# LIU-YUXI/SA-GNN

Hardware: AMD Instinct MI355X
Metric: spmm_edges_per_sec (higher is better)
Workload: dtype f32

## Files before the change

### include/sagnn.h

```cpp
#ifndef SAGNN_H
#define SAGNN_H

#include <stddef.h>
#include <stdint.h>

#ifdef __cplusplus
extern "C" {
#endif

#define SAGNN_VERSION 10400

enum {
  SAGNN_OK = 0,
  SAGNN_ERR_NULL = -1,
  SAGNN_ERR_DIM = -2,
  SAGNN_ERR_ALIGN = -3,
  SAGNN_ERR_CSR = -4,
  SAGNN_ERR_ARG = -5,
  SAGNN_ERR_WORKSPACE = -6,
  SAGNN_ERR_NOMEM = -7
};

int sagnn_version(void);

enum { SAGNN_ENGINE_F16X2 = 0, SAGNN_ENGINE_F32 = 1, SAGNN_ENGINE_VALU = 2 };
int sagnn_set_engine(int engine);
int sagnn_get_engine(void);
int sagnn_range_redo_count(int64_t* count, int reset);

size_t sagnn_last_error(char* buf, size_t cap);

int sagnn_profile_enable(int capacity);
int sagnn_profile_read(float* ms, int32_t* kind, int64_t* units_a, int64_t* units_b, int cap,
                       int* n_out);

int sagnn_csr_check_host(const int32_t* h_rowptr, const int32_t* h_colidx,
                         int64_t n_rows, int64_t n_src, int64_t nnz);

typedef struct sagnn_spmm_plan sagnn_spmm_plan;

typedef struct sagnn_spmm_tuning {
  int32_t short_thresh;
  int32_t long_thresh;
  int32_t chunk_edges;
  int32_t reserved;
} sagnn_spmm_tuning;

typedef struct sagnn_spmm_plan_info {
  int64_t n_rows, n_src, nnz;
  int64_t n_long_rows;
  int64_t n_chunks;
  int32_t short_thresh, long_thresh, chunk_edges;
  int32_t max_degree;
  int32_t on_device;
  int32_t weighted;
} sagnn_spmm_plan_info;

int sagnn_spmm_plan_create(const int32_t* h_rowptr, const int32_t* d_rowptr,
                           const int32_t* d_colidx, int64_t n_rows, int64_t n_src,
                           int64_t nnz, const sagnn_spmm_tuning* tuning ,
                           sagnn_spmm_plan** plan_out);
int sagnn_spmm_plan_destroy(sagnn_spmm_plan* plan);
int sagnn_spmm_plan_get_info(const sagnn_spmm_plan* plan, sagnn_spmm_plan_info* info);
int sagnn_spmm_plan_copy_chunks(const sagnn_spmm_plan* plan, int32_t* rows, int32_t* e_begin,
                                int32_t* e_end, int64_t cap);
int sagnn_spmm_plan_set_weights(sagnn_spmm_plan* plan, const float* d_weights);
size_t sagnn_spmm_workspace_bytes(const sagnn_spmm_plan* plan, int d);

int sagnn_spmm_f32(const sagnn_spmm_plan* plan, const float* X, int64_t ldx, int d,
                   const float* residual, int64_t ldr, float leaky, float* out, int64_t ldo,
                   const float* acc_in, int64_t ld_acc_in, float* acc_out, int64_t ld_acc_out,
                   void* workspace, size_t workspace_bytes, void* stream);

typedef struct sagnn_spmm_epilogue {
  float leaky;
  const float* residual; int64_t ldr;
  float* out; int64_t ldo;
  const float* acc_in; int64_t ld_acc_in;
  float* acc_out; int64_t ld_acc_out;
  uint8_t* mask_out;
  const uint8_t* mask_in;
  float* out2; int64_t ldo2; float slope2;
  const float* acc_in2; int64_t ld_acc_in2;
} sagnn_spmm_epilogue;

int sagnn_spmm_ex_f32(const sagnn_spmm_plan* plan, const float* X, int64_t ldx, int d,
                      const sagnn_spmm_epilogue* epilogue, void* workspace, size_t workspace_bytes,
                      void* stream);
int sagnn_mask_scale_f32(const float* g, int64_t ldg, const uint8_t* mask, float slope, float* out, int64_t ldo,
                         int64_t n_rows, int d, void* stream);

typedef struct sagnn_spmm_batch sagnn_spmm_batch;
int sagnn_spmm_batch_create(const sagnn_spmm_plan* const* plans_user, const sagnn_spmm_plan* const* plans_item,
                            int n_intervals, sagnn_spmm_batch** batch_out);
int sagnn_spmm_batch_destroy(sagnn_spmm_batch* batch);
size_t sagnn_spmm_batch_workspace_bytes(const sagnn_spmm_batch* batch, int d);

typedef struct sagnn_edge_drop {
  uint64_t seed;
  uint32_t step;
  uint32_t keep_threshold;
  float scale;
} sagnn_edge_drop;

int sagnn_spmm_drop_f32(const sagnn_spmm_plan* plan, const float* X, int64_t ldx, int d,
                        const sagnn_spmm_epilogue* epilogue, const sagnn_edge_drop* drop, uint32_t tag,
                        int rows_are_users, void* workspace, size_t workspace_bytes, void* stream);

int sagnn_spmm_plan_set_buckets(sagnn_spmm_plan* plan, const uint16_t* d_buckets, int32_t n_buckets);

typedef struct sagnn_edge_time {
  const float* te;
  int64_t stride_interval;
  int64_t stride_layer;
  int64_t stride_dir;
  int32_t n_buckets;
  float* dte;
  const sagnn_spmm_plan* adj_user;
  const sagnn_spmm_plan* adj_item;
  const sagnn_spmm_batch* adj_batch;
  void* adj_workspace;
  size_t adj_workspace_bytes;
} sagnn_edge_time;

int sagnn_spmm_time_batch_create(const sagnn_spmm_plan* const* adj_user, const sagnn_spmm_plan* const* adj_item,
                                 int n_intervals, sagnn_spmm_batch** batch_out);

int sagnn_spmm_time_f32(const sagnn_spmm_plan* plan, const float* X, int64_t ldx, int d,
                        const sagnn_spmm_epilogue* epilogue, const sagnn_edge_drop* drop, const sagnn_edge_time* time,
                        void* workspace, size_t workspace_bytes, void* stream);

typedef struct sagnn_gnn_side {
  const float* in;   int64_t ld_in,  slab_in;
  float*       out;  int64_t ld_out, slab_out;
  float*       scratch;
  uint8_t*     mask;
} sagnn_gnn_side;

enum { SAGNN_EDGES_PLAIN = 0, SAGNN_EDGES_DROP = 1, SAGNN_EDGES_TIME = 2 };

typedef struct sagnn_gnn_args {
  sagnn_gnn_side user, item;
  int d, n_layers;
  float leaky;
  int edges;
  const sagnn_edge_drop* drop;
  const sagnn_edge_time* time;
  int interval;
  void* workspace; size_t workspace_bytes;
} sagnn_gnn_args;

int sagnn_gnn_interval_f32(const sagnn_spmm_plan* plan_user, const sagnn_spmm_plan* plan_item, const sagnn_gnn_args* args,
                           void* stream);
int sagnn_gnn_interval_bwd_f32(const sagnn_spmm_plan* plan_user, const sagnn_spmm_plan* plan_item,
                               const sagnn_gnn_args* args, void* stream);
int sagnn_gnn_stack_f32(const sagnn_spmm_batch* batch, const sagnn_gnn_args* args, void* stream);
int sagnn_gnn_stack_bwd_f32(const sagnn_spmm_batch* batch, const sagnn_gnn_args* args, void* stream);

int sagnn_lstm_fwd_f32(const float* x, int64_t ld_n, int64_t ld_t, int64_t n, int t, int d, const float* W,
                       const float* b, float forget_bias, const float* drop_scale, float* h,
                       int64_t ld_h, void* stream);
int sagnn_lstm_fwd_state_f32(const float* x, int64_t ld_n, int64_t ld_t, int64_t n, int t, int d,
                             const float* W, const float* b, float forget_bias, const float* drop_scale,
                             const float* h_init, int64_t ld_hi, const float* c_init, float* h, int64_t ld_h,
                             float* c_final, void* stream);
int sagnn_layernorm_td_f32(const float* x, int64_t ld_n, int64_t ld_t, int64_t n, int t, int d,
                           const float* gamma, const float* beta, float eps, float* y,
                           int64_t ld_y, void* stream);
int sagnn_mhsa_mean_f32(const float* x, int64_t ld_n, int64_t ld_t, int64_t n, int t, int d, int heads,
                        const float* Wq, const float* bq, const float* Wk, const float* bk,
                        const float* Wv, const float* bv, float* out, int64_t ld_out,
                        void* stream);
size_t sagnn_mhsa_wide_workspace_bytes(int64_t n, int t, int d);
int sagnn_mhsa_mean_wide_f32(const float* x, int64_t ld_n, int64_t ld_t, int64_t n, int t, int d, int heads,
                             const float* Wq, const float* bq, const float* Wk, const float* bk, const float* Wv,
                             const float* bv, float* out, int64_t ld_out, void* workspace, size_t workspace_bytes,
                             void* stream);
size_t sagnn_ln_mhsa_mean_workspace_bytes(int64_t n, int t, int d, int heads);
int sagnn_ln_mhsa_mean_f32(const float* x, int64_t ld_n, int64_t ld_t, int64_t n, int t, int d, int heads,
                           const float* ln_gamma, const float* ln_beta, float ln_eps, const float* Wq,
                           const float* bq, const float* Wk, const float* bk, const float* Wv, const float* bv,
                           float* out, int64_t ld_out, void* workspace, size_t workspace_bytes, void* stream);
int sagnn_interval_fusion_f32(const float* x, int64_t ld_n, int64_t ld_t, int64_t n, int t, int d, int heads,
                              const float* lstm_W, const float* lstm_b, float forget_bias,
                              const float* ln_gamma, const float* ln_beta, float ln_eps,
                              const float* Wq, const float* bq, const float* Wk, const float* bk,
                              const float* Wv, const float* bv, float* out, int64_t ld_out,
                              void* workspace, size_t workspace_bytes, void* stream);
size_t sagnn_interval_fusion_workspace_bytes(int64_t n, int t, int d);

int sagnn_lstm_fwd_train_f32(const float* x, int64_t ld_n, int64_t ld_t, int64_t n, int t, int d,
                             const float* W, const float* b, float forget_bias, const float* drop_scale,
                             float* h, int64_t ld_h, float* gates, float* cell, void* stream);
int sagnn_attn_bwd_f32(float* qkv, const float* g_out, int64_t ld_g, int64_t n, int t, int d, int heads,
                       void* stream);
int sagnn_layernorm_td_bwd_f32(const float* h, int64_t ld_h, const float* dy, int64_t ld_dy, int64_t n, int t,
                               int d, const float* gamma, float eps, float* dh, int64_t ld_dh, float* dgamma,
                               float* dbeta, void* stream);
int sagnn_lstm_bwd_step_f32(const float* gates, const float* cell, const float* dh_ext, int64_t ld_dhe,
                            const float* drop_scale, const float* dh_rec, int64_t ld_dhr, const float* dc_in,
                            float* dgates, float* dc_out, int64_t n, int t, int d, int ts, void* stream);
int sagnn_attn_bwd_front_supported(int d, int t, int heads);
int sagnn_attn_bwd_front_f32(const float* x, int64_t ld_n, int64_t ld_t, int64_t n, int t, int d, int heads,
                             const float* ln_gamma, const float* ln_beta, float ln_eps, int apply_ln,
                             const float* Wq, const float* bq, const float* Wk, const float* bk, const float* Wv,
                             const float* bv, const float* g_out, int64_t ld_g, float* dqkv, float* y_out,
                             void* stream);
int sagnn_attn_bwd_tail_supported(int d);
int sagnn_attn_bwd_tail_f32(float* y, const float* dqkv, int64_t rows, int d, const float* Wqkv, float* dWqkv,
                            float* dbqkv, void* stream);
int sagnn_lstm_bwd_supported(int d);
int sagnn_lstm_bwd_f32(const float* x, int64_t ld_n, int64_t ld_t, const float* h, const float* gates,
                       const float* cell, const float* dh_ext, int64_t ld_dhe, const float* drop_scale,
                       const float* W, float* dx, float* dW, float* db, int64_t n, int t, int d, void* stream);
size_t sagnn_lstm_bwd_workspace_bytes(int64_t n, int t, int d);
int sagnn_lstm_bwd_ws_f32(const float* x, int64_t ld_n, int64_t ld_t, const float* h, const float* gates,
                          const float* cell, const float* dh_ext, int64_t ld_dhe, const float* drop_scale,
                          const float* W, float* dx, float* dW, float* db, int64_t n, int t, int d, void* workspace,
                          size_t workspace_bytes, void* stream);

int sagnn_leaky_add_f32(const float* a, const float* b, float* out, float leaky, int64_t count, void* stream);
int sagnn_pair_score_f32(const float* U, int64_t ldu, const float* I, int64_t ldi, const float* S, int64_t lds,
                         const float* A, int64_t lda, const int32_t* uids, const int32_t* iids,
                         const int32_t* locs, float leaky, float* out, int64_t n_pairs, int d, void* stream);

int sagnn_pair_score_bwd_f32(const float* U, int64_t ldu, const float* I, int64_t ldi, const float* S, int64_t lds,
                             const float* A, int64_t lda, const int32_t* uids, const int32_t* iids,
                             const int32_t* locs, float leaky, const float* g, float* dU, float* dI, float* dS,
                             float* dA, int64_t n_pairs, int d, void* stream);
int sagnn_prod_leaky_sum_f32(const float* X, int64_t ldx, const float* Y, int64_t ldy, const int32_t* uids,
                             const int32_t* iids, float leaky, float* out, int64_t n_pairs, int d, void* stream);
int sagnn_prod_leaky_sum_bwd_f32(const float* X, int64_t ldx, const float* Y, int64_t ldy, const int32_t* uids,
                                 const int32_t* iids, float leaky, const float* g, float* dX, float* dY,
                                 int64_t n_pairs, int d, void* stream);
int sagnn_meta_features_f32(const float* F, int64_t ldf, const float* V, int64_t ldv, const int32_t* uids,
                            float* out, int64_t n, int d, void* stream);
int sagnn_meta_features_bwd_f32(const float* F, int64_t ldf, const float* V, int64_t ldv, const int32_t* uids,
                                const float* dm, float* dF, float* dV, int64_t n, int d, void* stream);
int sagnn_leaky_f32(const float* a, const float* g, float* out, float leaky, int64_t count, int backward,
                    void* stream);
int sagnn_rowdot_sigmoid_f32(const float* A, int64_t lda, const float* w3, const float* b3, float* out, int64_t n,
                             int k, void* stream);
int sagnn_rowdot_sigmoid_bwd_f32(const float* A, int64_t lda, const float* w3, const float* w, const float* dw,
                                 float* dA, int64_t ldda, float* dw3, float* db3, int64_t n, int k, void* stream);
int sagnn_hinge_f32(const float* pos, const float* neg, const float* wp, const float* wn, const float* sp,
                    const float* sn, float scale, float* loss, float* dpos, float* dneg, float* dwp, float* dwn,
                    int64_t n, void* stream);

int sagnn_mul_f32(const float* a, const float* b, float* out, int64_t count, void* stream);

int sagnn_adam_step_f32(float* param, const float* grad, float* m, float* v, int64_t count, float lr,
                        float beta1, float beta2, float eps, float l2, int64_t step, void* stream);

int sagnn_adam_multi_f32(int n_tensors, float* const* params, const float* const* grads, float* const* m,
                         float* const* v, const int64_t* counts, const float* l2, float lr, float beta1,
                         float beta2, float eps, int64_t step, void* stream);

int sagnn_dense_nn_f32(const float* X, int64_t ldx, int64_t n, int din, int dout, const float* W,
                       const float* bias, float* Y, int64_t ldy, int accumulate, void* stream);
int sagnn_dense_tn_f32(const float* X, int64_t ldx, const float* G, int64_t ldg, int64_t n, int din,
                       int dout, float* dW, float* db, void* stream);
int sagnn_dense_tn_seg_f32(const float* X, int64_t ldx, int64_t x_seg, const float* G, int64_t ldg, int64_t g_seg,
                           int64_t seg_rows, int n_seg, int din, int dout, float* dW, float* db, void* stream);

size_t sagnn_score_topk_workspace_bytes(int64_t n_queries, int64_t n_items, int d, int k);
int sagnn_score_topk_f32(const float* Q, int64_t ldq, const float* I, int64_t ldi, int64_t n_queries, int64_t n_items,
                         int d, int k, const int32_t* excl_rowptr, const int32_t* excl_items, const int32_t* target,
                         int32_t* topk_items, float* topk_scores, int64_t* target_rank, void* workspace,
                         size_t workspace_bytes, void* stream);

int sagnn_candidate_rank_f32(const float* U, int64_t ldu, const float* I, int64_t ldi, const float* S, int64_t lds,
                             const float* A, int64_t lda, const int32_t* uids, const int32_t* cand, int64_t ldc,
                             const int32_t* target, float leaky, int64_t n_rows, int C, int d, int64_t* rank,
                             float* scores, int64_t ld_scores, void* stream);

int sagnn_sample_train_i32(const int32_t* bat_ids, int64_t n_batch, int64_t n_slots, const int64_t* seq_ptr,
                           const int32_t* seq_items, const int64_t* ban_ptr, const int32_t* ban_items, int64_t n_users,
                           int64_t n_items, int train_sample_num, int pred_num, int pos_length, const int64_t* pair_off,
                           int64_t n_pairs, uint64_t seed, int64_t step, int32_t* uids, int32_t* iids,
                           int32_t* uLocs_seq, int64_t* seg_begin, int32_t* seg_len, void* stream);
int sagnn_sample_ssl_i32(const int32_t* bat_ids, int64_t n_batch, int n_intervals, const int64_t* sub_ptr,
                         const int32_t* sub_items, int64_t n_users, int ssl_num, const int64_t* ssl_off, int64_t n_out,
                         uint64_t seed, int64_t step, int32_t* uids, int32_t* iids, int32_t* uLocs_seq, void* stream);
int sagnn_seq_sum_f32(const float* fi, int64_t ldf, int64_t n_items, const float* pos_embed, int64_t ldp,
                      int pos_length, const int32_t* seq_items, int64_t n_flat, const int64_t* seg_begin,
                      const int32_t* seg_len, int64_t n_slots, int d, float* seq_tok, float* pos_tok, int64_t ldo,
                      void* stream);
int sagnn_seq_sum_bwd_f32(const float* g_seq, const float* g_pos, int64_t ldg, const int32_t* seq_items, int64_t n_flat,
                          const int64_t* seg_begin, const int32_t* seg_len, int64_t n_slots, int pos_length, int d,
                          float* d_fi, int64_t ld_dfi, int64_t n_items, float* d_pos, int64_t ld_dpos, void* stream);

int sagnn_rows_mark_i32(const int32_t* ids, int64_t n_ids, int64_t n_rows, uint8_t* flags, void* stream);
int sagnn_rows_mark_seg_i32(const int32_t* seq_items, int64_t n_flat, const int64_t* seg_begin, const int32_t* seg_len,
                            int64_t n_slots, int max_len, int64_t n_rows, uint8_t* flags, void* stream);
size_t sagnn_rows_compact_workspace_bytes(int64_t n_rows);
int sagnn_rows_compact_i32(uint8_t* flags, int64_t n_rows, int32_t* rows, int64_t cap, int32_t* count, void* workspace,
                           size_t workspace_bytes, void* stream);
int sagnn_rows_gather_f32(const float* x, int64_t ld_n, int64_t ld_t, int64_t n_rows, int t, int d, const int32_t* rows,
                          int64_t cap, const int32_t* count, float* out, void* stream);
int sagnn_rows_scatter_f32(const float* src, const int32_t* rows, int64_t cap, const int32_t* count, int t, int d,
                           float* dst, int64_t ld_n, int64_t ld_t, int64_t n_rows, void* stream);

int sagnn_seq_attn_supported(int d, int heads, int pos_length);
int sagnn_seq_gather_f32(const float* fi, int64_t ldf, int64_t n_items, const float* pos_embed, int64_t ldp,
                         int pos_length, const int32_t* seq_items, int64_t n_flat, const int32_t* seq_pos,
                         const int64_t* seg_begin, const int32_t* seg_len, int64_t n_slots, int d, float* seq_slab,
                         float* pos_slab, int64_t ldo, void* stream);
int sagnn_seq_gather_bwd_f32(const float* g_seq, const float* g_pos, int64_t ldg, const int32_t* seq_items,
                             int64_t n_flat, const int32_t* seq_pos, const int64_t* seg_begin, const int32_t* seg_len,
                             int64_t n_slots, int pos_length, int d, float* d_fi, int64_t ld_dfi, int64_t n_items,
                             float* d_pos, int64_t ld_dpos, void* stream);
int sagnn_seq_attn_f32(const float* qkv, const int32_t* seg_len, int64_t n_slots, int pos_length, int d, int heads,
                       float* ctx, void* stream);
int sagnn_seq_attn_bwd_f32(const float* qkv, const float* g_ctx, const int32_t* seg_len, int64_t n_slots,
                           int pos_length, int d, int heads, float* dqkv, void* stream);
int sagnn_seq_pool_f32(const float* x, int64_t ldx, const int32_t* seg_len, int64_t n_slots, int pos_length, int d,
                       float* out, int64_t ldo, void* stream);
int sagnn_seq_pool_bwd_f32(const float* g, int64_t ldg, const int32_t* seg_len, int64_t n_slots, int pos_length, int d,
                           float* dx, int64_t ldx, void* stream);

size_t sagnn_softmax_loss_workspace_bytes(int64_t n_queries, int64_t n_items, int d);
int sagnn_softmax_loss_f32(const float* Q, int64_t ldq, const float* I, int64_t ldi, int64_t n_queries, int64_t n_items,
                           int d, const int32_t* target, float inv_temp, float scale, const int64_t* excl_ptr,
                           const int32_t* excl_items, const int32_t* excl_row, int64_t n_lists, float* loss, float* lse,
                           float* tscore, void* workspace, size_t workspace_bytes, void* stream);
int sagnn_softmax_loss_bwd_f32(const float* Q, int64_t ldq, const float* I, int64_t ldi, int64_t n_queries,
                               int64_t n_items, int d, const int32_t* target, float inv_temp, float scale,
                               const int64_t* excl_ptr, const int32_t* excl_items, const int32_t* excl_row,
                               int64_t n_lists, const float* lse, const float* g, float* dQ, int64_t lddq, float* dI,
                               int64_t lddi, void* workspace, size_t workspace_bytes, void* stream);

#ifdef __cplusplus
}
#endif
#endif
```

### sa-gnn_amd/_lib.py

```python
from __future__ import annotations

import ctypes
import os
from ctypes import POINTER, c_char_p, c_float, c_int, c_int32, c_int64, c_size_t, c_uint32, c_uint64, c_void_p

_HERE = os.path.dirname(os.path.abspath(__file__))
LIB_PATH = os.environ.get("SAGNN_LIB") or os.path.join(_HERE, "lib", "libsagnn.so")


class SagnnError(RuntimeError):
    def __init__(self, code: int, msg: str):
        super().__init__(f"libsagnn error {code}: {msg}")
        self.code = code


class Tuning(ctypes.Structure):
    _fields_ = [("short_thresh", c_int32), ("long_thresh", c_int32), ("chunk_edges", c_int32),
                ("reserved", c_int32)]


class SpmmEpilogue(ctypes.Structure):
    _fields_ = [("leaky", c_float), ("residual", c_void_p), ("ldr", c_int64), ("out", c_void_p),
                ("ldo", c_int64), ("acc_in", c_void_p), ("ld_acc_in", c_int64), ("acc_out", c_void_p),
                ("ld_acc_out", c_int64), ("mask_out", c_void_p), ("mask_in", c_void_p),
                ("out2", c_void_p), ("ldo2", c_int64), ("slope2", c_float), ("acc_in2", c_void_p),
                ("ld_acc_in2", c_int64)]


class EdgeDropArgs(ctypes.Structure):
    _fields_ = [("seed", c_uint64), ("step", c_uint32), ("keep_threshold", c_uint32), ("scale", c_float)]


class EdgeTimeArgs(ctypes.Structure):
    _fields_ = [("te", c_void_p), ("stride_interval", c_int64), ("stride_layer", c_int64), ("stride_dir", c_int64),
                ("n_buckets", c_int32), ("dte", c_void_p), ("adj_user", c_void_p), ("adj_item", c_void_p),
                ("adj_batch", c_void_p), ("adj_workspace", c_void_p), ("adj_workspace_bytes", c_size_t)]


class GnnSide(ctypes.Structure):
    _fields_ = [("in_", c_void_p), ("ld_in", c_int64), ("slab_in", c_int64), ("out", c_void_p), ("ld_out", c_int64),
                ("slab_out", c_int64), ("scratch", c_void_p), ("mask", c_void_p)]


EDGES_PLAIN, EDGES_DROP, EDGES_TIME = 0, 1, 2


class GnnArgs(ctypes.Structure):
    _fields_ = [("user", GnnSide), ("item", GnnSide), ("d", c_int), ("n_layers", c_int), ("leaky", c_float),
                ("edges", c_int), ("drop", POINTER(EdgeDropArgs)), ("time", POINTER(EdgeTimeArgs)), ("interval", c_int),
                ("workspace", c_void_p), ("workspace_bytes", c_size_t)]


class PlanInfo(ctypes.Structure):
    _fields_ = [("n_rows", c_int64), ("n_src", c_int64), ("nnz", c_int64),
                ("n_long_rows", c_int64), ("n_chunks", c_int64), ("short_thresh", c_int32),
                ("long_thresh", c_int32), ("chunk_edges", c_int32), ("max_degree", c_int32),
                ("on_device", c_int32), ("weighted", c_int32)]


SIGNATURES = {
    "sagnn_version": (c_int, []),
    "sagnn_set_engine": (c_int, [c_int]),
    "sagnn_get_engine": (c_int, []),
    "sagnn_range_redo_count": (c_int, [POINTER(c_int64), c_int]),
    "sagnn_last_error": (c_size_t, [c_char_p, c_size_t]),
    "sagnn_profile_enable": (c_int, [c_int]),
    "sagnn_profile_read": (c_int, [c_void_p, c_void_p, c_void_p, c_void_p, c_int, POINTER(c_int)]),
    "sagnn_csr_check_host": (c_int, [c_void_p, c_void_p, c_int64, c_int64, c_int64]),
    "sagnn_spmm_plan_create": (c_int, [c_void_p, c_void_p, c_void_p, c_int64, c_int64, c_int64,
                                       POINTER(Tuning), POINTER(c_void_p)]),
    "sagnn_spmm_plan_destroy": (c_int, [c_void_p]),
    "sagnn_spmm_plan_get_info": (c_int, [c_void_p, POINTER(PlanInfo)]),
    "sagnn_spmm_plan_set_weights": (c_int, [c_void_p, c_void_p]),
    "sagnn_spmm_plan_copy_chunks": (c_int, [c_void_p, c_void_p, c_void_p, c_void_p, c_int64]),
    "sagnn_spmm_workspace_bytes": (c_size_t, [c_void_p, c_int]),
    "sagnn_spmm_f32": (c_int, [c_void_p, c_void_p, c_int64, c_int, c_void_p, c_int64, c_float,
                               c_void_p, c_int64, c_void_p, c_int64, c_void_p, c_int64, c_void_p,
                               c_size_t, c_void_p]),
    "sagnn_spmm_ex_f32": (c_int, [c_void_p, c_void_p, c_int64, c_int, POINTER(SpmmEpilogue), c_void_p, c_size_t,
                                  c_void_p]),
    "sagnn_mask_scale_f32": (c_int, [c_void_p, c_int64, c_void_p, c_float, c_void_p, c_int64, c_int64, c_int, c_void_p]),
    "sagnn_spmm_batch_create": (c_int, [c_void_p, c_void_p, c_int, POINTER(c_void_p)]),
    "sagnn_spmm_batch_destroy": (c_int, [c_void_p]),
    "sagnn_spmm_batch_workspace_bytes": (c_size_t, [c_void_p, c_int]),
    "sagnn_gnn_interval_f32": (c_int, [c_void_p, c_void_p, POINTER(GnnArgs), c_void_p]),
    "sagnn_gnn_interval_bwd_f32": (c_int, [c_void_p, c_void_p, POINTER(GnnArgs), c_void_p]),
    "sagnn_gnn_stack_f32": (c_int, [c_void_p, POINTER(GnnArgs), c_void_p]),
    "sagnn_gnn_stack_bwd_f32": (c_int, [c_void_p, POINTER(GnnArgs), c_void_p]),
    "sagnn_spmm_drop_f32": (c_int, [c_void_p, c_void_p, c_int64, c_int, POINTER(SpmmEpilogue), POINTER(EdgeDropArgs),
                                    c_uint32, c_int, c_void_p, c_size_t, c_void_p]),
    "sagnn_spmm_plan_set_buckets": (c_int, [c_void_p, c_void_p, c_int32]),
    "sagnn_spmm_time_batch_create": (c_int, [c_void_p, c_void_p, c_int, POINTER(c_void_p)]),
    "sagnn_spmm_time_f32": (c_int, [c_void_p, c_void_p, c_int64, c_int, POINTER(SpmmEpilogue), POINTER(EdgeDropArgs),
                                    POINTER(EdgeTimeArgs), c_void_p, c_size_t, c_void_p]),
    "sagnn_lstm_fwd_train_f32": (c_int, [c_void_p, c_int64, c_int64, c_int64, c_int, c_int, c_void_p, c_void_p, c_float,
                                         c_void_p, c_void_p, c_int64, c_void_p, c_void_p, c_void_p]),
    "sagnn_mhsa_wide_workspace_bytes": (c_size_t, [c_int64, c_int, c_int]),
    "sagnn_ln_mhsa_mean_workspace_bytes": (c_size_t, [c_int64, c_int, c_int, c_int]),
    "sagnn_ln_mhsa_mean_f32": (c_int, [c_void_p, c_int64, c_int64, c_int64, c_int, c_int, c_int, c_void_p, c_void_p,
                                       c_float, c_void_p, c_void_p, c_void_p, c_void_p, c_void_p, c_void_p, c_void_p,
                                       c_int64, c_void_p, c_size_t, c_void_p]),
    "sagnn_mhsa_mean_wide_f32": (c_int, [c_void_p, c_int64, c_int64, c_int64, c_int, c_int, c_int, c_void_p, c_void_p,
                                         c_void_p, c_void_p, c_void_p, c_void_p, c_void_p, c_int64, c_void_p, c_size_t,
                                         c_void_p]),
    "sagnn_attn_bwd_f32": (c_int, [c_void_p, c_void_p, c_int64, c_int64, c_int, c_int, c_int, c_void_p]),
    "sagnn_layernorm_td_bwd_f32": (c_int, [c_void_p, c_int64, c_void_p, c_int64, c_int64, c_int, c_int, c_void_p,
                                           c_float, c_void_p, c_int64, c_void_p, c_void_p, c_void_p]),
    "sagnn_lstm_bwd_step_f32": (c_int, [c_void_p, c_void_p, c_void_p, c_int64, c_void_p, c_void_p, c_int64, c_void_p,
                                        c_void_p, c_void_p, c_int64, c_int, c_int, c_int, c_void_p]),
    "sagnn_attn_bwd_front_supported": (c_int, [c_int, c_int, c_int]),
    "sagnn_attn_bwd_front_f32": (c_int, [c_void_p, c_int64, c_int64, c_int64, c_int, c_int, c_int, c_void_p, c_void_p,
                                         c_float, c_int, c_void_p, c_void_p, c_void_p, c_void_p, c_void_p, c_void_p,
                                         c_void_p, c_int64, c_void_p, c_void_p, c_void_p]),
    "sagnn_attn_bwd_tail_supported": (c_int, [c_int]),
    "sagnn_attn_bwd_tail_f32": (c_int, [c_void_p, c_void_p, c_int64, c_int, c_void_p, c_void_p, c_void_p, c_void_p]),
    "sagnn_lstm_bwd_supported": (c_int, [c_int]),
    "sagnn_lstm_bwd_f32": (c_int, [c_void_p, c_int64, c_int64, c_void_p, c_void_p, c_void_p, c_void_p, c_int64, c_void_p,
                                   c_void_p, c_void_p, c_void_p, c_void_p, c_int64, c_int, c_int, c_void_p]),
    "sagnn_lstm_bwd_workspace_bytes": (c_size_t, [c_int64, c_int, c_int]),
    "sagnn_lstm_bwd_ws_f32": (c_int, [c_void_p, c_int64, c_int64, c_void_p, c_void_p, c_void_p, c_void_p, c_int64, c_void_p,
                                      c_void_p, c_void_p, c_void_p, c_void_p, c_int64, c_int, c_int, c_void_p, c_size_t, c_void_p]),
    "sagnn_leaky_add_f32": (c_int, [c_void_p, c_void_p, c_void_p, c_float, c_int64, c_void_p]),
    "sagnn_pair_score_f32": (c_int, [c_void_p, c_int64, c_void_p, c_int64, c_void_p, c_int64, c_void_p, c_int64,
                                     c_void_p, c_void_p, c_void_p, c_float, c_void_p, c_int64, c_int, c_void_p]),
    "sagnn_pair_score_bwd_f32": (c_int, [c_void_p, c_int64, c_void_p, c_int64, c_void_p, c_int64, c_void_p, c_int64,
                                         c_void_p, c_void_p, c_void_p, c_float, c_void_p, c_void_p, c_void_p, c_void_p,
                                         c_void_p, c_int64, c_int, c_void_p]),
    "sagnn_prod_leaky_sum_f32": (c_int, [c_void_p, c_int64, c_void_p, c_int64, c_void_p, c_void_p, c_float, c_void_p,
                                         c_int64, c_int, c_void_p]),
    "sagnn_prod_leaky_sum_bwd_f32": (c_int, [c_void_p, c_int64, c_void_p, c_int64, c_void_p, c_void_p, c_float,
                                             c_void_p, c_void_p, c_void_p, c_int64, c_int, c_void_p]),
    "sagnn_meta_features_f32": (c_int, [c_void_p, c_int64, c_void_p, c_int64, c_void_p, c_void_p, c_int64, c_int,
                                        c_void_p]),
    "sagnn_meta_features_bwd_f32": (c_int, [c_void_p, c_int64, c_void_p, c_int64, c_void_p, c_void_p, c_void_p,
                                            c_void_p, c_int64, c_int, c_void_p]),
    "sagnn_leaky_f32": (c_int, [c_void_p, c_void_p, c_void_p, c_float, c_int64, c_int, c_void_p]),
    "sagnn_rowdot_sigmoid_f32": (c_int, [c_void_p, c_int64, c_void_p, c_void_p, c_void_p, c_int64, c_int, c_void_p]),
    "sagnn_rowdot_sigmoid_bwd_f32": (c_int, [c_void_p, c_int64, c_void_p, c_void_p, c_void_p, c_void_p, c_int64,
                                             c_void_p, c_void_p, c_int64, c_int, c_void_p]),
    "sagnn_hinge_f32": (c_int, [c_void_p, c_void_p, c_void_p, c_void_p, c_void_p, c_void_p, c_float, c_void_p,
                                c_void_p, c_void_p, c_void_p, c_void_p, c_int64, c_void_p]),
    "sagnn_mul_f32": (c_int, [c_void_p, c_void_p, c_void_p, c_int64, c_void_p]),
    "sagnn_adam_step_f32": (c_int, [c_void_p, c_void_p, c_void_p, c_void_p, c_int64, c_float, c_float, c_float,
                                    c_float, c_float, c_int64, c_void_p]),
    "sagnn_adam_multi_f32": (c_int, [c_int, c_void_p, c_void_p, c_void_p, c_void_p, c_void_p, c_void_p, c_float, c_float,
                                     c_float, c_float, c_int64, c_void_p]),
    "sagnn_dense_nn_f32": (c_int, [c_void_p, c_int64, c_int64, c_int, c_int, c_void_p, c_void_p, c_void_p, c_int64,
                                   c_int, c_void_p]),
    "sagnn_dense_tn_f32": (c_int, [c_void_p, c_int64, c_void_p, c_int64, c_int64, c_int, c_int, c_void_p, c_void_p,
                                   c_void_p]),
    "sagnn_dense_tn_seg_f32": (c_int, [c_void_p, c_int64, c_int64, c_void_p, c_int64, c_int64, c_int64, c_int, c_int, c_int,
                                       c_void_p, c_void_p, c_void_p]),
    "sagnn_lstm_fwd_f32": (c_int, [c_void_p, c_int64, c_int64, c_int64, c_int, c_int, c_void_p, c_void_p,
                                   c_float, c_void_p, c_void_p, c_int64, c_void_p]),
    "sagnn_lstm_fwd_state_f32": (c_int, [c_void_p, c_int64, c_int64, c_int64, c_int, c_int, c_void_p, c_void_p, c_float,
                                         c_void_p, c_void_p, c_int64, c_void_p, c_void_p, c_int64, c_void_p, c_void_p]),
    "sagnn_layernorm_td_f32": (c_int, [c_void_p, c_int64, c_int64, c_int64, c_int, c_int, c_void_p, c_void_p,
                                       c_float, c_void_p, c_int64, c_void_p]),
    "sagnn_mhsa_mean_f32": (c_int, [c_void_p, c_int64, c_int64, c_int64, c_int, c_int, c_int, c_void_p,
                                    c_void_p, c_void_p, c_void_p, c_void_p, c_void_p, c_void_p,
                                    c_int64, c_void_p]),
    "sagnn_interval_fusion_f32": (c_int, [c_void_p, c_int64, c_int64, c_int64, c_int, c_int, c_int, c_void_p,
                                          c_void_p, c_float, c_void_p, c_void_p, c_float, c_void_p,
                                          c_void_p, c_void_p, c_void_p, c_void_p, c_void_p, c_void_p,
                                          c_int64, c_void_p, c_size_t, c_void_p]),
    "sagnn_interval_fusion_workspace_bytes": (c_size_t, [c_int64, c_int, c_int]),
    "sagnn_score_topk_workspace_bytes": (c_size_t, [c_int64, c_int64, c_int, c_int]),
    "sagnn_score_topk_f32": (c_int, [c_void_p, c_int64, c_void_p, c_int64, c_int64, c_int64, c_int, c_int, c_void_p,
                                     c_void_p, c_void_p, c_void_p, c_void_p, c_void_p, c_void_p, c_size_t, c_void_p]),
    "sagnn_candidate_rank_f32": (c_int, [c_void_p, c_int64, c_void_p, c_int64, c_void_p, c_int64, c_void_p, c_int64,
                                         c_void_p, c_void_p, c_int64, c_void_p, c_float, c_int64, c_int, c_int, c_void_p,
                                         c_void_p, c_int64, c_void_p]),
    "sagnn_sample_train_i32": (c_int, [c_void_p, c_int64, c_int64, c_void_p, c_void_p, c_void_p, c_void_p, c_int64, c_int64,
                                       c_int, c_int, c_int, c_void_p, c_int64, c_uint64, c_int64, c_void_p, c_void_p,
                                       c_void_p, c_void_p, c_void_p, c_void_p]),
    "sagnn_sample_ssl_i32": (c_int, [c_void_p, c_int64, c_int, c_void_p, c_void_p, c_int64, c_int, c_void_p, c_int64,
                                     c_uint64, c_int64, c_void_p, c_void_p, c_void_p, c_void_p]),
    "sagnn_seq_sum_f32": (c_int, [c_void_p, c_int64, c_int64, c_void_p, c_int64, c_int, c_void_p, c_int64, c_void_p,
                                  c_void_p, c_int64, c_int, c_void_p, c_void_p, c_int64, c_void_p]),
    "sagnn_seq_sum_bwd_f32": (c_int, [c_void_p, c_void_p, c_int64, c_void_p, c_int64, c_void_p, c_void_p, c_int64, c_int,
                                      c_int, c_void_p, c_int64, c_int64, c_void_p, c_int64, c_void_p]),
    "sagnn_rows_mark_i32": (c_int, [c_void_p, c_int64, c_int64, c_void_p, c_void_p]),
    "sagnn_rows_mark_seg_i32": (c_int, [c_void_p, c_int64, c_void_p, c_void_p, c_int64, c_int, c_int64, c_void_p, c_void_p]),
    "sagnn_rows_compact_workspace_bytes": (c_size_t, [c_int64]),
    "sagnn_rows_compact_i32": (c_int, [c_void_p, c_int64, c_void_p, c_int64, c_void_p, c_void_p, c_size_t, c_void_p]),
    "sagnn_rows_gather_f32": (c_int, [c_void_p, c_int64, c_int64, c_int64, c_int, c_int, c_void_p, c_int64, c_void_p,
                                      c_void_p, c_void_p]),
    "sagnn_rows_scatter_f32": (c_int, [c_void_p, c_void_p, c_int64, c_void_p, c_int, c_int, c_void_p, c_int64, c_int64,
                                       c_int64, c_void_p]),
    "sagnn_seq_attn_supported": (c_int, [c_int, c_int, c_int]),
    "sagnn_seq_gather_f32": (c_int, [c_void_p, c_int64, c_int64, c_void_p, c_int64, c_int, c_void_p, c_int64, c_void_p,
                                     c_void_p, c_void_p, c_int64, c_int, c_void_p, c_void_p, c_int64, c_void_p]),
    "sagnn_seq_gather_bwd_f32": (c_int, [c_void_p, c_void_p, c_int64, c_void_p, c_int64, c_void_p, c_void_p, c_void_p,
                                         c_int64, c_int, c_int, c_void_p, c_int64, c_int64, c_void_p, c_int64, c_void_p]),
    "sagnn_seq_attn_f32": (c_int, [c_void_p, c_void_p, c_int64, c_int, c_int, c_int, c_void_p, c_void_p]),
    "sagnn_seq_attn_bwd_f32": (c_int, [c_void_p, c_void_p, c_void_p, c_int64, c_int, c_int, c_int, c_void_p, c_void_p]),
    "sagnn_seq_pool_f32": (c_int, [c_void_p, c_int64, c_void_p, c_int64, c_int, c_int, c_void_p, c_int64, c_void_p]),
    "sagnn_seq_pool_bwd_f32": (c_int, [c_void_p, c_int64, c_void_p, c_int64, c_int, c_int, c_void_p, c_int64, c_void_p]),
    "sagnn_softmax_loss_workspace_bytes": (c_size_t, [c_int64, c_int64, c_int]),
    "sagnn_softmax_loss_f32": (c_int, [c_void_p, c_int64, c_void_p, c_int64, c_int64, c_int64, c_int, c_void_p, c_float,
                                       c_float, c_void_p, c_void_p, c_void_p, c_int64, c_void_p, c_void_p, c_void_p,
                                       c_void_p, c_size_t, c_void_p]),
    "sagnn_softmax_loss_bwd_f32": (c_int, [c_void_p, c_int64, c_void_p, c_int64, c_int64, c_int64, c_int, c_void_p, c_float,
                                           c_float, c_void_p, c_void_p, c_void_p, c_int64, c_void_p, c_void_p, c_void_p,
                                           c_int64, c_void_p, c_int64, c_void_p, c_size_t, c_void_p]),
}


_lib = None


def load() -> ctypes.CDLL:
    global _lib
    if _lib is not None:
        return _lib
    if not os.path.exists(LIB_PATH):
        raise ImportError(
            f"{LIB_PATH} not found: build it with `python -c 'import __graft_entry__ as g; "
            "g.build()'` (or `make -C sa-gnn_amd/csrc`). There is no fallback path.")
    lib = ctypes.CDLL(LIB_PATH)
    lib.sagnn_version.restype = c_int
    if lib.sagnn_version() < 10400:
        raise ImportError(f"{LIB_PATH} is libsagnn {lib.sagnn_version()}: this binding needs >= 10400 (sagnn_gnn_args)")
    for name, (res, args) in SIGNATURES.items():
        fn = getattr(lib, name)
        fn.restype = res
        fn.argtypes = args
    _lib = lib
    return lib


def last_error() -> str:
    buf = ctypes.create_string_buffer(1024)
    load().sagnn_last_error(buf, 1024)
    return buf.value.decode("utf-8", "replace")


def check(rc: int) -> None:
    if rc != 0:
        raise SagnnError(rc, last_error())
```

### sa-gnn_amd/csrc/spmm.hip

```cpp
#include <float.h>

#include <algorithm>
#include <new>
#include <type_traits>
#include <vector>

#include "common.h"
#include "philox.h"

namespace {

constexpr int kWave = 64;
constexpr int kBlock = 256;
constexpr int kWavesPerBlock = kBlock / kWave;
constexpr int kRowsPerWave = 16;
constexpr int64_t kSmallRows = 262144;
constexpr int kUnroll = 8;

struct Epilogue {
  const float* residual;
  int64_t ldr;
  const float* acc_in;
  int64_t ld_acc_in;
  float* out;
  int64_t ldo;
  float* acc_out;
  int64_t ld_acc_out;
  float leaky;
  uint8_t* mask_out;
  const uint8_t* mask_in;
  float* out2;
  int64_t ldo2;
  float slope2;
  int mask_stride;
  const float* acc_in2;
  int64_t ld_acc_in2;
};

__device__ __forceinline__ float4 ld4(const float* p) {
  return *reinterpret_cast<const float4*>(p);
}
__device__ __forceinline__ void st4(float* p, float4 v) { *reinterpret_cast<float4*>(p) = v; }
typedef float f32x4_t __attribute__((ext_vector_type(4)));
__device__ __forceinline__ float4 ld4s(const float* p) {
#ifndef SAGNN_PLAIN_STREAMS
  const f32x4_t v = __builtin_nontemporal_load(reinterpret_cast<const f32x4_t*>(p));
  return make_float4(v.x, v.y, v.z, v.w);
#else
  return ld4(p);
#endif
}
__device__ __forceinline__ void st4s(float* p, float4 v) {
#ifndef SAGNN_PLAIN_STREAMS
  const f32x4_t w = {v.x, v.y, v.z, v.w};
  __builtin_nontemporal_store(w, reinterpret_cast<f32x4_t*>(p));
#else
  st4(p, v);
#endif
}
__device__ __forceinline__ int ldi_s(const int32_t* p) {
#ifndef SAGNN_PLAIN_STREAMS
  return __builtin_nontemporal_load(p);
#else
  return *p;
#endif
}
__device__ __forceinline__ float ldf_s(const float* p) {
#ifndef SAGNN_PLAIN_STREAMS
  return __builtin_nontemporal_load(p);
#else
  return *p;
#endif
}
__device__ __forceinline__ int ldb_s(const uint16_t* p) {
#ifndef SAGNN_PLAIN_STREAMS
  return __builtin_nontemporal_load(p);
#else
  return *p;
#endif
}
__device__ __forceinline__ void add4(float4& a, const float4& b) {
  a.x += b.x;
  a.y += b.y;
  a.z += b.z;
  a.w += b.w;
}

struct RowDrop {
  uint32_t k0, k1, step, thresh, tag;
  int rows_users;
  float scale;
};
struct BatchDrop {
  RowDrop r;
  uint32_t tag_i;
};

__device__ __forceinline__ RowDrop seg_drop(const BatchDrop& b, int dir, int k) {
  RowDrop r = b.r;
  r.tag = (dir ? b.tag_i : r.tag) | ((uint32_t)k << 8);
  r.rows_users = !dir;
  return r;
}

template <bool WEIGHTED>
__device__ __forceinline__ void acc4(float4& a, float w, const float4& v) {
  if constexpr (WEIGHTED) {
    a.x = fmaf(w, v.x, a.x);
    a.y = fmaf(w, v.y, a.y);
    a.z = fmaf(w, v.z, a.z);
    a.w = fmaf(w, v.w, a.w);
  } else {
    add4(a, v);
  }
}

template <bool DROP>
__device__ __forceinline__ int keep_edge(const RowDrop& dr, int row, int idx) {
  if constexpr (DROP) {
    const uint32_t u = dr.rows_users ? (uint32_t)row : (uint32_t)idx;
    const uint32_t i = dr.rows_users ? (uint32_t)idx : (uint32_t)row;
    const sagnn::Word4 w = sagnn::philox4x32_10(sagnn::Word4{u, i, dr.tag, dr.step}, dr.k0, dr.k1);
    return w.x < dr.thresh ? idx : -1;
  } else {
    return idx;
  }
}

template <bool DROP>
__device__ __forceinline__ float4 drop_scale(const RowDrop& dr, float4 s) {
  if constexpr (DROP) return make_float4(dr.scale * s.x, dr.scale * s.y, dr.scale * s.z, dr.scale * s.w);
  else return s;
}

struct RowTime {
  const uint16_t* bucket;
  const float* te;
};
struct BatchTime {
  const uint16_t* const* buckets;
  const float* te;
  int64_t s_k, s_dir;
};
__device__ __forceinline__ RowTime seg_time(const BatchTime& t, int seg, int dir, int k) {
  return RowTime{t.buckets[seg], t.te + (int64_t)k * t.s_k + (int64_t)dir * t.s_dir};
}
__device__ __forceinline__ RowTime seg_time(const RowTime& t, int, int, int) { return t; }

template <class T>
struct KernelArg { using type = T; };
template <class T>
struct KernelArg<T*> { using type = T* __restrict__; };
template <class Want, class... A>
constexpr bool kHas = (std::is_same_v<Want, A> || ...);
template <class... A>
struct Pack {
  static constexpr bool DROP = kHas<RowDrop, A...> || kHas<BatchDrop, A...>;
  static constexpr bool WEIGHTED = kHas<const float*, A...> || kHas<const float* const*, A...>;
  static constexpr bool TIME = kHas<RowTime, A...> || kHas<BatchTime, A...>;
  static_assert(DROP == kHas<const int32_t*, A...>, "a drop comes with the rows of the chunks");
  static_assert(!(DROP && TIME), "there are no drop + time kernels");
  static_assert(sizeof...(A) == 2 * DROP + WEIGHTED + TIME, "trailing arguments: a drop, weights, a time term");
};
template <class Want>
__device__ __forceinline__ Want arg_of() { return Want{}; }
template <class Want, class A0, class... A>
__device__ __forceinline__ Want arg_of(A0 a0, A... rest) {
  if constexpr (std::is_same_v<Want, A0>) return a0;
  else return arg_of<Want, A...>(rest...);
}
template <class... A>
__device__ __forceinline__ int chunk_row_of(int64_t ci, A... da) {
  if constexpr (Pack<A...>::DROP) return arg_of<const int32_t*, A...>(da...)[ci];
  else return 0;
}
template <class... A>
__device__ __forceinline__ const float* weights_of(int seg, A... da) {
  if constexpr (kHas<const float* const*, A...>) return arg_of<const float* const*, A...>(da...)[seg];
  else return arg_of<const float*, A...>(da...);
}
__device__ __forceinline__ float4 scaled(float4 s) { return s; }
__device__ __forceinline__ float4 scaled(float4 s, float scale) {
  return make_float4(scale * s.x, scale * s.y, scale * s.z, scale * s.w);
}

__device__ __forceinline__ void finish_row(const Epilogue& ep, int64_t row, int col, float4 s) {
  float4 y;
  y.x = fmaxf(ep.leaky * s.x, s.x);
  y.y = fmaxf(ep.leaky * s.y, s.y);
  y.z = fmaxf(ep.leaky * s.z, s.z);
  y.w = fmaxf(ep.leaky * s.w, s.w);
  if (ep.mask_out) {
    const unsigned bits = (s.x > ep.leaky * s.x ? 1u : 0u) | (s.y > ep.leaky * s.y ? 2u : 0u) |
                          (s.z > ep.leaky * s.z ? 4u : 0u) | (s.w > ep.leaky * s.w ? 8u : 0u);
    ep.mask_out[row * ep.mask_stride + (col >> 2)] = (uint8_t)bits;
  }
  float4 r = make_float4(0.f, 0.f, 0.f, 0.f);
  if (ep.residual) {
    r = ld4s(ep.residual + row * ep.ldr + col);
    add4(y, r);
  }
  if (ep.out) st4s(ep.out + row * ep.ldo + col, y);
  if (ep.acc_out) {
    float4 a = make_float4(0.f, 0.f, 0.f, 0.f);
    if (ep.acc_in) {
      a = (ep.acc_in == ep.residual && ep.ld_acc_in == ep.ldr)
              ? r
              : ld4s(ep.acc_in + row * ep.ld_acc_in + col);
    }
    add4(a, y);
    if (ep.acc_in2) add4(a, ld4s(ep.acc_in2 + row * ep.ld_acc_in2 + col));
    st4s(ep.acc_out + row * ep.ld_acc_out + col, a);
    y = a;
  }
  if (ep.out2) {
    const unsigned bits = ep.mask_in ? ep.mask_in[row * ep.mask_stride + (col >> 2)] : 15u;
    float4 z;
    z.x = (bits & 1u) ? y.x : ep.slope2 * y.x;
    z.y = (bits & 2u) ? y.y : ep.slope2 * y.y;
    z.z = (bits & 4u) ? y.z : ep.slope2 * y.z;
    z.w = (bits & 8u) ? y.w : ep.slope2 * y.w;
    st4s(ep.out2 + row * ep.ldo2 + col, z);
  }
}

__global__ void mask_scale_kernel(const float* __restrict__ g, int64_t ldg, int64_t s_g, const uint8_t* __restrict__ mask,
                                  int64_t s_mask, int mask_stride, float slope, float* __restrict__ gm, int64_t ldgm,
                                  int64_t s_gm, int64_t n_rows, int d) {
  const int64_t i = (int64_t)blockIdx.x * blockDim.x + threadIdx.x;
  const int lpr = d >> 2;
  if (i >= n_rows * lpr) return;
  const int64_t k = blockIdx.y;
  const int64_t row = i / lpr;
  const int l = (int)(i - row * lpr);
  const float4 v = ld4(g + k * s_g + row * ldg + 4 * l);
  const unsigned bits = mask[k * s_mask + row * mask_stride + l];
  float4 z;
  z.x = (bits & 1u) ? v.x : slope * v.x;
  z.y = (bits & 2u) ? v.y : slope * v.y;
  z.z = (bits & 4u) ? v.z : slope * v.z;
  z.w = (bits & 8u) ? v.w : slope * v.w;
  st4(gm + k * s_gm + row * ldgm + 4 * l, z);
}

template <int LPR, bool IDENT, bool DROP = false, bool WEIGHTED = false, bool TIME = false>
__device__ __forceinline__ float4 wave_row_sum(const int32_t* __restrict__ colidx, int e0, int e1,
                                               const float* __restrict__ X, int64_t ldx,
                                               int lane, int grp, int col, bool lane_on, const RowDrop& dr = RowDrop{},
                                               int row = 0, const float* __restrict__ w = nullptr,
                                               const RowTime& tm = RowTime{}, int ldte = 0) {
  static_assert(!(IDENT && (WEIGHTED || TIME)), "the fix-up pass adds partial sums that carry the weights and the time term already");
  constexpr int G = kWave / LPR;
  constexpr int STEP = G * kUnroll;
  float4 acc = make_float4(0.f, 0.f, 0.f, 0.f);
  int idx_next = -1;
  float w_next = 0.f;
  int b_next = 0;
  if (e0 + lane < e1) {
    idx_next = IDENT ? (e0 + lane) : ldi_s(colidx + e0 + lane);
    if constexpr (WEIGHTED) w_next = ldf_s(w + e0 + lane);
    if constexpr (TIME) b_next = ldb_s(tm.bucket + e0 + lane);
  }
  for (int e = e0; e < e1; e += kWave) {
    const int idx = keep_edge<DROP>(dr, row, idx_next);
    const float wt = w_next;
    const int bk = b_next;
    const int en = e + kWave;
    idx_next = -1;
    if constexpr (WEIGHTED) w_next = 0.f;
    if constexpr (TIME) b_next = 0;
    if (en + lane < e1) {
      idx_next = IDENT ? (en + lane) : ldi_s(colidx + en + lane);
      if constexpr (WEIGHTED) w_next = ldf_s(w + en + lane);
      if constexpr (TIME) b_next = ldb_s(tm.bucket + en + lane);
    }
    const int cnt = min(kWave, e1 - e);
    for (int j = 0; j < cnt; j += STEP) {
      float4 v[kUnroll];
      int c[kUnroll];
      float cw[kUnroll];
      int cb[kUnroll];
#pragma unroll
      for (int u = 0; u < kUnroll; ++u) {
        c[u] = __shfl(idx, j + u * G + grp);
        if constexpr (WEIGHTED) cw[u] = __shfl(wt, j + u * G + grp);
        else cw[u] = 1.f;
        if constexpr (TIME) cb[u] = __shfl(bk, j + u * G + grp);
        else cb[u] = 0;
      }
#pragma unroll
      for (int u = 0; u < kUnroll; ++u) {
        v[u] = make_float4(0.f, 0.f, 0.f, 0.f);
        if (c[u] >= 0 && lane_on) v[u] = ld4(X + (int64_t)c[u] * ldx + col);
      }
      if constexpr (TIME) {
#pragma unroll
        for (int u = 0; u < kUnroll; ++u)
          if (c[u] >= 0 && lane_on) add4(v[u], ld4(tm.te + cb[u] * ldte + col));
      }
#pragma unroll
      for (int u = 0; u < kUnroll; ++u) acc4<WEIGHTED>(acc, cw[u], v[u]);
    }
  }
#pragma unroll
  for (int off = LPR; off < kWave; off <<= 1) {
    acc.x += __shfl_xor(acc.x, off);
    acc.y += __shfl_xor(acc.y, off);
    acc.z += __shfl_xor(acc.z, off);
    acc.w += __shfl_xor(acc.w, off);
  }
  return acc;
}

template <int LPR, int RPW, bool DROP, bool WEIGHTED, bool TIME = false>
__device__ __forceinline__ void rows_wave(const int32_t* __restrict__ rowptr, const int32_t* __restrict__ colidx,
                                          const float* __restrict__ X, int64_t ldx, int d, int64_t n_rows, int64_t row0,
                                          int short_t, int long_t, const Epilogue& ep, int lane,
                                          const RowDrop& dr, const float* __restrict__ w,
                                          const RowTime& tm = RowTime{}) {
  constexpr int G = kWave / LPR;
  const int grp = lane / LPR;
  const int sub = lane % LPR;
  const int col = 4 * sub;
  const bool lane_on = col < d;
  const int nr = (int)min((int64_t)RPW, n_rows - row0);
  const int rp = rowptr[row0 + min(lane, nr)];
  const int rp_up = __shfl_down(rp, 1);
  const int deg_l = (lane < nr) ? (rp_up - rp) : 0;
  unsigned long long medium = __ballot(deg_l > short_t && deg_l <= long_t);

  int e0_n = __shfl(rp, grp);
  int dg_n = __shfl(deg_l, grp);
  int idx_n = -1;
  float w_n = 0.f;
  int b_n = 0;
  if (dg_n <= short_t && sub < dg_n) {
    idx_n = ldi_s(colidx + e0_n + sub);
    if constexpr (WEIGHTED) w_n = ldf_s(w + e0_n + sub);
    if constexpr (TIME) b_n = ldb_s(tm.bucket + e0_n + sub);
  }
#pragma unroll 1
  for (int it = 0; it < RPW / G; ++it) {
    const int lr = it * G + grp;
    const int e0 = e0_n;
    const int dg = dg_n;
    int idx = keep_edge<DROP>(dr, (int)row0 + lr, idx_n);
    float wt = w_n;
    int bk = b_n;
    const bool mine = (lr < nr) && (dg <= short_t);
    const int my_deg = mine ? dg : 0;
    if (it + 1 < RPW / G) {
      e0_n = __shfl(rp, lr + G);
      dg_n = __shfl(deg_l, lr + G);
      idx_n = -1;
      if constexpr (WEIGHTED) w_n = 0.f;
      if constexpr (TIME) b_n = 0;
      if (dg_n <= short_t && sub < dg_n) {
        idx_n = ldi_s(colidx + e0_n + sub);
        if constexpr (WEIGHTED) w_n = ldf_s(w + e0_n + sub);
        if constexpr (TIME) b_n = ldb_s(tm.bucket + e0_n + sub);
      }
    }
    int maxdeg = 0;
#pragma unroll
    for (int g = 0; g < G; ++g) {
      const int x = __builtin_amdgcn_readlane(deg_l, it * G + g);
      maxdeg = max(maxdeg, x <= short_t ? x : 0);
    }
    float4 acc = make_float4(0.f, 0.f, 0.f, 0.f);
    for (int eo = 0; eo < maxdeg; eo += LPR) {
      if (eo > 0) {
        const int k = eo + sub;
        idx = (k < my_deg) ? keep_edge<DROP>(dr, (int)row0 + lr, ldi_s(colidx + e0 + k)) : -1;
        if constexpr (WEIGHTED) wt = (k < my_deg) ? ldf_s(w + e0 + k) : 0.f;
        if constexpr (TIME) bk = (k < my_deg) ? ldb_s(tm.bucket + e0 + k) : 0;
      }
      const int lim = min(LPR, maxdeg - eo);
      for (int j = 0; j < lim; j += kUnroll) {
        float4 v[kUnroll];
        int c[kUnroll];
        float cw[kUnroll];
        int cb[kUnroll];
#pragma unroll
        for (int u = 0; u < kUnroll; ++u) {
          c[u] = __shfl(idx, grp * LPR + j + u);
          if constexpr (WEIGHTED) cw[u] = __shfl(wt, grp * LPR + j + u);
          else cw[u] = 1.f;
          if constexpr (TIME) cb[u] = __shfl(bk, grp * LPR + j + u);
          else cb[u] = 0;
        }
#pragma unroll
        for (int u = 0; u < kUnroll; ++u) {
          v[u] = make_float4(0.f, 0.f, 0.f, 0.f);
          if (c[u] >= 0 && lane_on) v[u] = ld4(X + (int64_t)c[u] * ldx + col);
        }
        if constexpr (TIME) {
#pragma unroll
          for (int u = 0; u < kUnroll; ++u)
            if (c[u] >= 0 && lane_on) add4(v[u], ld4(tm.te + cb[u] * d + col));
        }
#pragma unroll
        for (int u = 0; u < kUnroll; ++u) acc4<WEIGHTED>(acc, cw[u], v[u]);
      }
    }
    if (mine && lane_on) finish_row(ep, row0 + lr, col, drop_scale<DROP>(dr, acc));
  }

  while (medium) {
    const int lr = __builtin_ctzll(medium);
    medium &= medium - 1;
    const int e0 = __builtin_amdgcn_readlane(rp, lr);
    const int dg = __builtin_amdgcn_readlane(deg_l, lr);
    const float4 s =
        wave_row_sum<LPR, false, DROP, WEIGHTED, TIME>(colidx, e0, e0 + dg, X, ldx, lane, grp, col, lane_on, dr, (int)row0 + lr, w,
                                                       tm, d);
    if (grp == 0 && lane_on) finish_row(ep, row0 + lr, col, drop_scale<DROP>(dr, s));
  }
}

template <int LPR, int RPW, class... DropArgs>
__global__ __launch_bounds__(kBlock) void spmm_rows_kernel(
    const int32_t* __restrict__ rowptr, const int32_t* __restrict__ colidx,
    const float* __restrict__ X, int64_t ldx, int d, int64_t n_rows, int short_t, int long_t,
    const int32_t* __restrict__ chunk_e0, const int32_t* __restrict__ chunk_e1, int64_t n_chunks,
    int chunk_blocks, float* __restrict__ partial, Epilogue ep, typename KernelArg<DropArgs>::type... da) {
  constexpr bool DROP = Pack<DropArgs...>::DROP, WEIGHTED = Pack<DropArgs...>::WEIGHTED, TIME = Pack<DropArgs...>::TIME;
  const int lane = threadIdx.x & (kWave - 1);
  const int wave = threadIdx.x / kWave;

  if ((int)blockIdx.x < chunk_blocks) {
    const int grp = lane / LPR;
    const int col = 4 * (lane % LPR);
    const bool lane_on = col < d;
    const int64_t ci = (int64_t)blockIdx.x * kWavesPerBlock + wave;
    if (ci >= n_chunks) return;
    const float4 s = wave_row_sum<LPR, false, DROP, WEIGHTED, TIME>(
        colidx, chunk_e0[ci], chunk_e1[ci], X, ldx, lane, grp, col, lane_on, arg_of<RowDrop, DropArgs...>(da...),
        chunk_row_of<DropArgs...>(ci, da...), weights_of<DropArgs...>(0, da...), arg_of<RowTime, DropArgs...>(da...), d);
    if (grp == 0 && lane_on) st4(partial + ci * (int64_t)d + col, s);
    return;
  }

  const int64_t row0 = ((int64_t)(blockIdx.x - chunk_blocks) * kWavesPerBlock + wave) * RPW;
  if (row0 >= n_rows) return;
  rows_wave<LPR, RPW, DROP, WEIGHTED, TIME>(rowptr, colidx, X, ldx, d, n_rows, row0, short_t, long_t, ep, lane,
                                            arg_of<RowDrop, DropArgs...>(da...), weights_of<DropArgs...>(0, da...),
                                            arg_of<RowTime, DropArgs...>(da...));
}

template <int LPR, class... Scale>
__global__ __launch_bounds__(kBlock) void spmm_fixup_kernel(const int32_t* __restrict__ long_row,
                                                           const int32_t* __restrict__ long_slot,
                                                           int64_t n_long,
                                                           const float* __restrict__ partial, int d,
                                                           Epilogue ep, Scale... scale) {
  static_assert(sizeof...(Scale) <= 1, "drop-only argument: none, or the scale");
  const int lane = threadIdx.x & (kWave - 1);
  const int wave = threadIdx.x / kWave;
  const int grp = lane / LPR;
  const int col = 4 * (lane % LPR);
  const bool lane_on = col < d;
  const int64_t li = (int64_t)blockIdx.x * kWavesPerBlock + wave;
  if (li >= n_long) return;
  const float4 s = wave_row_sum<LPR, true>(nullptr, long_slot[li], long_slot[li + 1], partial, d,
                                           lane, grp, col, lane_on);
  if (grp == 0 && lane_on) finish_row(ep, long_row[li], col, scaled(s, scale...));
}

struct SegMeta {
  const int32_t* rowptr;
  const int32_t* colidx;
  int32_t short_t, long_t;
};
struct DirArgs {
  const float* X;
  int64_t ldx, s_X;
  Epilogue ep;
  int64_t s_res, s_acc_in, s_out, s_acc_out, s_mask_out, s_mask_in, s_out2, s_acc_in2;
};
struct BatchGeom {
  int32_t T;
  int32_t chunk_blocks;
  int32_t blocks_u, blocks_i;
  int32_t rows_u, rows_i;
};

__device__ __forceinline__ Epilogue seg_epilogue(const DirArgs& a, int k) {
  Epilogue e = a.ep;
  if (e.residual) e.residual += (int64_t)k * a.s_res;
  if (e.acc_in) e.acc_in += (int64_t)k * a.s_acc_in;
  if (e.out) e.out += (int64_t)k * a.s_out;
  if (e.acc_out) e.acc_out += (int64_t)k * a.s_acc_out;
  if (e.mask_out) e.mask_out += (int64_t)k * a.s_mask_out;
  if (e.mask_in) e.mask_in += (int64_t)k * a.s_mask_in;
  if (e.out2) e.out2 += (int64_t)k * a.s_out2;
  if (e.acc_in2) e.acc_in2 += (int64_t)k * a.s_acc_in2;
  return e;
}

template <int LPR, int RPW, class... DropArgs>
__global__ __launch_bounds__(kBlock) void spmm_rows_batch_kernel(const SegMeta* __restrict__ meta, BatchGeom g,
                                                                const int32_t* __restrict__ chunk_e0,
                                                                const int32_t* __restrict__ chunk_e1,
                                                                const int32_t* __restrict__ chunk_seg, int64_t n_chunks,
                                                                float* __restrict__ partial, int d, DirArgs au, DirArgs ai,
                                                                typename KernelArg<DropArgs>::type... da) {
  constexpr bool DROP = Pack<DropArgs...>::DROP, WEIGHTED = Pack<DropArgs...>::WEIGHTED, TIME = Pack<DropArgs...>::TIME;
  const int lane = threadIdx.x & (kWave - 1);
  const int wave = threadIdx.x / kWave;
  if ((int)blockIdx.x < g.chunk_blocks) {
    const int grp = lane / LPR;
    const int col = 4 * (lane % LPR);
    const bool lane_on = col < d;
    const int64_t ci = (int64_t)blockIdx.x * kWavesPerBlock + wave;
    if (ci >= n_chunks) return;
    const int seg = __builtin_amdgcn_readfirstlane(chunk_seg[ci]);
    const int dir = seg >= g.T, k = seg - dir * g.T;
    const DirArgs& a = dir ? ai : au;
    RowTime tm{};
    if constexpr (TIME) tm = seg_time(arg_of<BatchTime, DropArgs...>(da...), seg, dir, k);
    const float4 s = wave_row_sum<LPR, false, DROP, WEIGHTED, TIME>(
        meta[seg].colidx, chunk_e0[ci], chunk_e1[ci], a.X + (int64_t)k * a.s_X, a.ldx, lane, grp, col, lane_on,
        seg_drop(arg_of<BatchDrop, DropArgs...>(da...), dir, k), chunk_row_of<DropArgs...>(ci, da...),
        weights_of<DropArgs...>(seg, da...), tm, d);
    if (grp == 0 && lane_on) st4(partial + ci * (int64_t)d + col, s);
    return;
  }
  int rb = (int)blockIdx.x - g.chunk_blocks;
  const int dir = rb >= g.T * g.blocks_u;
  if (dir) rb -= g.T * g.blocks_u;
  const int per = dir ? g.blocks_i : g.blocks_u;
  const int k = rb / per;
  const int64_t n_rows = dir ? g.rows_i : g.rows_u;
  const int64_t row0 = ((int64_t)(rb - k * per) * kWavesPerBlock + wave) * RPW;
  if (row0 >= n_rows) return;
  const SegMeta m = meta[dir * g.T + k];
  const DirArgs& a = dir ? ai : au;
  const Epilogue ep = seg_epilogue(a, k);
  RowTime tm{};
  if constexpr (TIME) tm = seg_time(arg_of<BatchTime, DropArgs...>(da...), dir * g.T + k, dir, k);
  rows_wave<LPR, RPW, DROP, WEIGHTED, TIME>(m.rowptr, m.colidx, a.X + (int64_t)k * a.s_X, a.ldx, d, n_rows, row0, m.short_t,
                                            m.long_t, ep, lane, seg_drop(arg_of<BatchDrop, DropArgs...>(da...), dir, k),
                                            weights_of<DropArgs...>(dir * g.T + k, da...), tm);
}

template <int LPR, class... Scale>
__global__ __launch_bounds__(kBlock) void spmm_fixup_batch_kernel(const int32_t* __restrict__ long_row,
                                                                 const int32_t* __restrict__ long_slot,
                                                                 const int32_t* __restrict__ long_seg, int64_t n_long,
                                                                 const float* __restrict__ partial, int d, int T,
                                                                 DirArgs au, DirArgs ai, Scale... scale) {
  static_assert(sizeof...(Scale) <= 1, "drop-only argument: none, or the scale");
  const int lane = threadIdx.x & (kWave - 1);
  const int wave = threadIdx.x / kWave;
  const int grp = lane / LPR;
  const int col = 4 * (lane % LPR);
  const bool lane_on = col < d;
  const int64_t li = (int64_t)blockIdx.x * kWavesPerBlock + wave;
  if (li >= n_long) return;
  const int seg = __builtin_amdgcn_readfirstlane(long_seg[li]);
  const int dir = seg >= T, k = seg - dir * T;
  const Epilogue ep = seg_epilogue(dir ? ai : au, k);
  const float4 s = wave_row_sum<LPR, true>(nullptr, long_slot[li], long_slot[li + 1], partial, d, lane, grp, col, lane_on);
  if (grp == 0 && lane_on) finish_row(ep, long_row[li], col, scaled(s, scale...));
}

}

struct sagnn_spmm_plan {
  sagnn_spmm_plan_info info{};
  const int32_t* d_rowptr = nullptr;
  const int32_t* d_colidx = nullptr;
  std::vector<int32_t> chunk_row, chunk_e0, chunk_e1;
  std::vector<int32_t> long_row, long_slot;
  int32_t* d_meta = nullptr;
  const int32_t *d_chunk_e0 = nullptr, *d_chunk_e1 = nullptr, *d_long_row = nullptr,
                *d_long_slot = nullptr, *d_chunk_row = nullptr;
  const float* d_weights = nullptr;
  const uint16_t* d_buckets = nullptr;
  int32_t n_buckets = 0;
};

namespace {
constexpr int kDefaultShort = 16;
constexpr int kDefaultLong = 256;
constexpr int kDefaultChunk = 256;

int check_rowptr(const int32_t* rp, int64_t n_rows, int64_t nnz) {
  if (rp[0] != 0) return sagnn::fail(SAGNN_ERR_CSR, "rowptr[0] = %d, expected 0", rp[0]);
  for (int64_t r = 0; r < n_rows; ++r)
    if (rp[r + 1] < rp[r])
      return sagnn::fail(SAGNN_ERR_CSR, "rowptr decreases at row %lld", (long long)r);
  if (rp[n_rows] != nnz)
    return sagnn::fail(SAGNN_ERR_CSR, "rowptr[n_rows] = %d but nnz = %lld", rp[n_rows],
                       (long long)nnz);
  return SAGNN_OK;
}
}

extern "C" int sagnn_csr_check_host(const int32_t* h_rowptr, const int32_t* h_colidx,
                                    int64_t n_rows, int64_t n_src, int64_t nnz) {
  if (!h_rowptr || (nnz > 0 && !h_colidx)) return sagnn::fail(SAGNN_ERR_NULL, "null CSR array");
  if (n_rows < 0 || n_src < 0 || nnz < 0 || nnz > INT32_MAX || n_rows >= INT32_MAX ||
      n_src > INT32_MAX)
    return sagnn::fail(SAGNN_ERR_ARG, "CSR sizes out of int32 range");
  if (int rc = check_rowptr(h_rowptr, n_rows, nnz)) return rc;
  for (int64_t e = 0; e < nnz; ++e)
    if (h_colidx[e] < 0 || h_colidx[e] >= n_src)
      return sagnn::fail(SAGNN_ERR_CSR, "colidx[%lld] = %d outside [0, %lld)", (long long)e,
                         h_colidx[e], (long long)n_src);
  return SAGNN_OK;
}

extern "C" int sagnn_spmm_plan_create(const int32_t* h_rowptr, const int32_t* d_rowptr,
                                      const int32_t* d_colidx, int64_t n_rows, int64_t n_src,
                                      int64_t nnz, const sagnn_spmm_tuning* tuning,
                                      sagnn_spmm_plan** plan_out) {
  if (!plan_out) return sagnn::fail(SAGNN_ERR_NULL, "plan_out is NULL");
  *plan_out = nullptr;
  if (!h_rowptr) return sagnn::fail(SAGNN_ERR_NULL, "h_rowptr is NULL");
  if ((d_rowptr == nullptr) != (d_colidx == nullptr) && nnz > 0)
    return sagnn::fail(SAGNN_ERR_NULL, "d_rowptr and d_colidx must both be given or both NULL");
  if (n_rows < 0 || n_src < 0 || nnz < 0 || nnz > INT32_MAX - 256 || n_rows >= INT32_MAX - 256 ||
      n_src > INT32_MAX)
    return sagnn::fail(SAGNN_ERR_ARG, "CSR sizes out of int32 range");
  if (int rc = check_rowptr(h_rowptr, n_rows, nnz)) return rc;

  sagnn_spmm_plan* p = new (std::nothrow) sagnn_spmm_plan();
  if (!p) return sagnn::fail(SAGNN_ERR_NOMEM, "out of host memory");
  int short_t = tuning && tuning->short_thresh > 0 ? tuning->short_thresh : kDefaultShort;
  int long_t = tuning && tuning->long_thresh > 0 ? tuning->long_thresh : kDefaultLong;
  int chunk = tuning && tuning->chunk_edges > 0 ? tuning->chunk_edges : kDefaultChunk;
  chunk = (chunk + kWave - 1) / kWave * kWave;
  if (long_t < short_t) long_t = short_t;

  int32_t max_deg = 0;
  try {
    p->long_slot.push_back(0);
    for (int64_t r = 0; r < n_rows; ++r) {
      const int32_t b = h_rowptr[r], e = h_rowptr[r + 1], deg = e - b;
      max_deg = std::max(max_deg, deg);
      if (deg <= long_t) continue;
      const int32_t nck = (deg + chunk - 1) / chunk;
      int32_t len = (deg + nck - 1) / nck;
      len = (len + kWave - 1) / kWave * kWave;
      for (int32_t s = b; s < e; s += len) {
        p->chunk_row.push_back((int32_t)r);
        p->chunk_e0.push_back(s);
        p->chunk_e1.push_back(std::min(e, s + len));
      }
      p->long_row.push_back((int32_t)r);
      p->long_slot.push_back((int32_t)p->chunk_row.size());
    }
  } catch (const std::bad_alloc&) {
    delete p;
    return sagnn::fail(SAGNN_ERR_NOMEM, "out of host memory building chunk list");
  }

  p->info.n_rows = n_rows;
  p->info.n_src = n_src;
  p->info.nnz = nnz;
  p->info.n_long_rows = (int64_t)p->long_row.size();
  p->info.n_chunks = (int64_t)p->chunk_row.size();
  p->info.short_thresh = short_t;
  p->info.long_thresh = long_t;
  p->info.chunk_edges = chunk;
  p->info.max_degree = max_deg;
  p->info.on_device = 0;
  p->d_rowptr = d_rowptr;
  p->d_colidx = d_colidx;

  if (d_rowptr) {
    const size_t nck = p->chunk_row.size(), nl = p->long_row.size();
    if (nck > 0) {
      const size_t words = 3 * nck + nl + (nl + 1);
      hipError_t e = hipMalloc((void**)&p->d_meta, words * sizeof(int32_t));
      if (e != hipSuccess) {
        delete p;
        return sagnn::hip_fail(e, "hipMalloc(plan metadata)");
      }
      std::vector<int32_t> host(words);
      std::copy(p->chunk_e0.begin(), p->chunk_e0.end(), host.begin());
      std::copy(p->chunk_e1.begin(), p->chunk_e1.end(), host.begin() + nck);
      std::copy(p->long_row.begin(), p->long_row.end(), host.begin() + 2 * nck);
      std::copy(p->long_slot.begin(), p->long_slot.end(), host.begin() + 2 * nck + nl);
      std::copy(p->chunk_row.begin(), p->chunk_row.end(), host.begin() + 2 * nck + 2 * nl + 1);
      e = hipMemcpy(p->d_meta, host.data(), words * sizeof(int32_t), hipMemcpyHostToDevice);
      if (e != hipSuccess) {
        (void)hipFree(p->d_meta);
        delete p;
        return sagnn::hip_fail(e, "hipMemcpy(plan metadata)");
      }
      p->d_chunk_e0 = p->d_meta;
      p->d_chunk_e1 = p->d_meta + nck;
      p->d_long_row = p->d_meta + 2 * nck;
      p->d_long_slot = p->d_meta + 2 * nck + nl;
      p->d_chunk_row = p->d_meta + 2 * nck + 2 * nl + 1;
    }
    p->info.on_device = 1;
  }
  *plan_out = p;
  return SAGNN_OK;
}

extern "C" int sagnn_spmm_plan_destroy(sagnn_spmm_plan* plan) {
  if (!plan) return SAGNN_OK;
  if (plan->d_meta) (void)hipFree(plan->d_meta);
  delete plan;
  return SAGNN_OK;
}

extern "C" int sagnn_spmm_plan_set_weights(sagnn_spmm_plan* plan, const float* d_weights) {
  if (!plan) return sagnn::fail(SAGNN_ERR_NULL, "plan is NULL");
  if (!plan->info.on_device) return sagnn::fail(SAGNN_ERR_ARG, "plan was built host-only (no device CSR): it takes no weights");
  if (d_weights && (reinterpret_cast<uintptr_t>(d_weights) & 3))
    return sagnn::fail(SAGNN_ERR_ALIGN, "weights: pointer must be 4-byte aligned");
  plan->d_weights = d_weights;
  plan->info.weighted = d_weights ? 1 : 0;
  return SAGNN_OK;
}

extern "C" int sagnn_spmm_plan_set_buckets(sagnn_spmm_plan* plan, const uint16_t* d_buckets, int32_t n_buckets) {
  if (!plan) return sagnn::fail(SAGNN_ERR_NULL, "plan is NULL");
  if (!plan->info.on_device) return sagnn::fail(SAGNN_ERR_ARG, "plan was built host-only (no device CSR): it takes no buckets");
  if (d_buckets && (n_buckets < 1 || n_buckets > 65535))
    return sagnn::fail(SAGNN_ERR_ARG, "buckets: n_buckets = %d, need 1 <= n_buckets <= 65535 (uint16 ids)", n_buckets);
  if (d_buckets && (reinterpret_cast<uintptr_t>(d_buckets) & 1))
    return sagnn::fail(SAGNN_ERR_ALIGN, "buckets: pointer must be 2-byte aligned");
  plan->d_buckets = d_buckets;
  plan->n_buckets = d_buckets ? n_buckets : 0;
  return SAGNN_OK;
}

extern "C" int sagnn_spmm_plan_get_info(const sagnn_spmm_plan* plan, sagnn_spmm_plan_info* info) {
  if (!plan || !info) return sagnn::fail(SAGNN_ERR_NULL, "plan/info is NULL");
  *info = plan->info;
  return SAGNN_OK;
}

extern "C" int sagnn_spmm_plan_copy_chunks(const sagnn_spmm_plan* plan, int32_t* rows,
                                           int32_t* e_begin, int32_t* e_end, int64_t cap) {
  if (!plan) return sagnn::fail(SAGNN_ERR_NULL, "plan is NULL");
  const int64_t n = plan->info.n_chunks;
  if (cap < n) return sagnn::fail(SAGNN_ERR_ARG, "cap %lld < n_chunks %lld", (long long)cap, (long long)n);
  if (n > 0 && (!rows || !e_begin || !e_end)) return sagnn::fail(SAGNN_ERR_NULL, "null output array");
  std::copy(plan->chunk_row.begin(), plan->chunk_row.end(), rows);
  std::copy(plan->chunk_e0.begin(), plan->chunk_e0.end(), e_begin);
  std::copy(plan->chunk_e1.begin(), plan->chunk_e1.end(), e_end);
  return SAGNN_OK;
}

extern "C" size_t sagnn_spmm_workspace_bytes(const sagnn_spmm_plan* plan, int d) {
  if (!plan || d <= 0) return 0;
  return (size_t)plan->info.n_chunks * (size_t)d * sizeof(float);
}

namespace {

template <int LPR>
int launch_spmm(const sagnn_spmm_plan* p, const float* X, int64_t ldx, int d, const Epilogue& ep,
                float* partial, hipStream_t stream, const RowDrop* drop = nullptr, const float* te = nullptr) {
  const int64_t n_rows = p->info.n_rows;
  const int64_t n_chunks = p->info.n_chunks;
  const int64_t chunk_blocks = (n_chunks + kWavesPerBlock - 1) / kWavesPerBlock;
  constexpr int G = kWave / LPR;
  constexpr int RPW_SMALL = G > 4 ? G : 4;
  const bool small = n_rows < kSmallRows;
  const int64_t rows_per_block = (int64_t)kWavesPerBlock * (small ? RPW_SMALL : kRowsPerWave);
  const int64_t row_blocks = (n_rows + rows_per_block - 1) / rows_per_block;
  const int64_t blocks = chunk_blocks + row_blocks;
  if (blocks > INT32_MAX) return sagnn::fail(SAGNN_ERR_ARG, "grid too large");
  if (blocks > 0) {
    sagnn::ProfileScope prof(sagnn::kProfSpmmRows, stream, p->info.nnz, n_rows);
    const auto rows = [&](auto kernel, auto... da) {
      hipLaunchKernelGGL(kernel, dim3((unsigned)blocks), dim3(kBlock), 0, stream, p->d_rowptr, p->d_colidx, X, ldx, d, n_rows,
                         p->info.short_thresh, p->info.long_thresh, p->d_chunk_e0, p->d_chunk_e1, n_chunks,
                         (int)chunk_blocks, partial, ep, da...);
    };
    const float* w = p->d_weights;
    const RowTime tm{p->d_buckets, te};
    if (te && w)
      rows(small ? spmm_rows_kernel<LPR, RPW_SMALL, RowTime, const float*> : spmm_rows_kernel<LPR, kRowsPerWave, RowTime, const float*>,
           tm, w);
    else if (te)
      rows(small ? spmm_rows_kernel<LPR, RPW_SMALL, RowTime> : spmm_rows_kernel<LPR, kRowsPerWave, RowTime>, tm);
    else if (drop && w)
      rows(small ? spmm_rows_kernel<LPR, RPW_SMALL, const int32_t*, RowDrop, const float*>
                 : spmm_rows_kernel<LPR, kRowsPerWave, const int32_t*, RowDrop, const float*>,
           p->d_chunk_row, *drop, w);
    else if (drop)
      rows(small ? spmm_rows_kernel<LPR, RPW_SMALL, const int32_t*, RowDrop> : spmm_rows_kernel<LPR, kRowsPerWave, const int32_t*, RowDrop>,
           p->d_chunk_row, *drop);
    else if (w)
      rows(small ? spmm_rows_kernel<LPR, RPW_SMALL, const float*> : spmm_rows_kernel<LPR, kRowsPerWave, const float*>, w);
    else
      rows(small ? spmm_rows_kernel<LPR, RPW_SMALL> : spmm_rows_kernel<LPR, kRowsPerWave>);
    SAGNN_HIP_TRY(hipGetLastError());
  }
  const int64_t n_long = p->info.n_long_rows;
  if (n_long > 0) {
    sagnn::ProfileScope prof(sagnn::kProfSpmmFixup, stream, n_chunks, n_long);
    const int64_t fb = (n_long + kWavesPerBlock - 1) / kWavesPerBlock;
    const auto fixup = [&](auto kernel, auto... scale) {
      hipLaunchKernelGGL(kernel, dim3((unsigned)fb), dim3(kBlock), 0, stream,
                         p->d_long_row, p->d_long_slot, n_long, partial, d, ep, scale...);
    };
    if (drop) fixup(spmm_fixup_kernel<LPR, float>, drop->scale);
    else fixup(spmm_fixup_kernel<LPR>);
    SAGNN_HIP_TRY(hipGetLastError());
  }
  return SAGNN_OK;
}

int check_mat(const char* name, const void* ptr, int64_t ld, int d, bool required) {
  if (!ptr) return required ? sagnn::fail(SAGNN_ERR_NULL, "%s is NULL", name) : SAGNN_OK;
  if (!sagnn::aligned16(ptr) || (ld & 3) != 0)
    return sagnn::fail(SAGNN_ERR_ALIGN, "%s: pointer must be 16-byte aligned and ld a multiple of 4", name);
  if (ld < d) return sagnn::fail(SAGNN_ERR_ARG, "%s: ld %lld < d %d", name, (long long)ld, d);
  return SAGNN_OK;
}

int check_d(int d) {
  if (d < 4 || d > 256 || (d & 3)) return sagnn::fail(SAGNN_ERR_DIM, "d = %d: need a multiple of 4 in [4, 256]", d);
  return SAGNN_OK;
}

struct Slab {
  float* p;
  int64_t ld, slab;
};

int check_slab(const char* name, const Slab& x, int d) {
  if (int rc = check_mat(name, x.p, x.ld, d, true)) return rc;
  if (x.slab & 3) return sagnn::fail(SAGNN_ERR_ALIGN, "%s: slab stride must be a multiple of 4", name);
  return SAGNN_OK;
}

int launch_mask_scale(const Slab& g, const uint8_t* mask, int64_t s_mask, float slope, const Slab& out, int64_t n_rows,
                      int d, int64_t T, hipStream_t stream) {
  const int64_t n = n_rows * (d / 4);
  if (n == 0) return SAGNN_OK;
  hipLaunchKernelGGL(mask_scale_kernel, dim3((unsigned)((n + 255) / 256), (unsigned)T), dim3(256), 0, stream, g.p, g.ld,
                     g.slab, mask, s_mask, d / 4, slope, out.p, out.ld, out.slab, n_rows, d);
  SAGNN_HIP_TRY(hipGetLastError());
  return SAGNN_OK;
}

Epilogue kernel_epilogue(const sagnn_spmm_epilogue& e, int d) {
  return Epilogue{e.residual, e.ldr,      e.acc_in,  e.ld_acc_in, e.out,  e.ldo,    e.acc_out, e.ld_acc_out,
                  e.leaky,    e.mask_out, e.mask_in, e.out2,      e.ldo2, e.slope2, d / 4,     e.acc_in2,
                  e.ld_acc_in2};
}

int spmm_ex(const sagnn_spmm_plan* plan, const float* X, int64_t ldx, int d, const Epilogue& e, void* workspace,
            size_t workspace_bytes, void* stream, const RowDrop* drop = nullptr, const float* te = nullptr) {
  if (!plan->info.on_device) return sagnn::fail(SAGNN_ERR_ARG, "plan was built host-only (no device CSR)");
  if (int rc = check_d(d)) return rc;
  if (te) {
    if (drop) return sagnn::fail(SAGNN_ERR_ARG, "edge time: no product takes a drop and a time term");
    if (!plan->d_buckets) return sagnn::fail(SAGNN_ERR_ARG, "edge time: the plan has no buckets (sagnn_spmm_plan_set_buckets)");
    if (!sagnn::aligned16(te)) return sagnn::fail(SAGNN_ERR_ALIGN, "edge time: TE must be 16-byte aligned");
  }
  if (!e.out && !e.acc_out && !e.out2) return sagnn::fail(SAGNN_ERR_NULL, "no output given");
  if (int rc = check_mat("X", X, ldx, d, plan->info.nnz > 0)) return rc;
  if (int rc = check_mat("residual", e.residual, e.ldr, d, false)) return rc;
  if (int rc = check_mat("out", e.out, e.ldo, d, false)) return rc;
  if (int rc = check_mat("acc_in", e.acc_in, e.ld_acc_in, d, false)) return rc;
  if (int rc = check_mat("acc_out", e.acc_out, e.ld_acc_out, d, false)) return rc;
  if (int rc = check_mat("acc_in2", e.acc_in2, e.ld_acc_in2, d, false)) return rc;
  if (e.acc_in2 && !e.acc_out) return sagnn::fail(SAGNN_ERR_ARG, "acc_in2 given without acc_out");
  if (int rc = check_mat("out2", e.out2, e.ldo2, d, false)) return rc;
  if ((e.out && e.out == X) || (e.acc_out && e.acc_out == X) || (e.out2 && e.out2 == X))
    return sagnn::fail(SAGNN_ERR_ARG, "outputs must not alias X");
  if (e.mask_in && !e.out2) return sagnn::fail(SAGNN_ERR_ARG, "mask_in given without out2");
  const size_t need = sagnn_spmm_workspace_bytes(plan, d);
  if (need > 0) {
    if (!workspace || workspace_bytes < need)
      return sagnn::fail(SAGNN_ERR_WORKSPACE, "workspace needs %zu bytes, got %zu", need,
                         workspace ? workspace_bytes : (size_t)0);
    if (!sagnn::aligned16(workspace)) return sagnn::fail(SAGNN_ERR_ALIGN, "workspace not 16-byte aligned");
  }
  if (plan->info.n_rows == 0) return SAGNN_OK;

  hipStream_t s = static_cast<hipStream_t>(stream);
  float* partial = static_cast<float*>(workspace);
  switch (sagnn::lanes_per_row(d)) {
    case 8: return launch_spmm<8>(plan, X, ldx, d, e, partial, s, drop, te);
    case 16: return launch_spmm<16>(plan, X, ldx, d, e, partial, s, drop, te);
    case 32: return launch_spmm<32>(plan, X, ldx, d, e, partial, s, drop, te);
    default: return launch_spmm<64>(plan, X, ldx, d, e, partial, s, drop, te);
  }
}

}

extern "C" int sagnn_spmm_ex_f32(const sagnn_spmm_plan* plan, const float* X, int64_t ldx, int d,
                                 const sagnn_spmm_epilogue* e, void* workspace, size_t workspace_bytes,
                                 void* stream) {
  if (!plan || !e) return sagnn::fail(SAGNN_ERR_NULL, "plan/epilogue is NULL");
  return spmm_ex(plan, X, ldx, d, kernel_epilogue(*e, d), workspace, workspace_bytes, stream);
}

namespace {
constexpr int kDropMaxLayers = 127;
constexpr int64_t kDropMaxIntervals = 1 << 23;

int check_drop(const sagnn_edge_drop* drop, int n_layers, int64_t last_interval) {
  if (!drop) return sagnn::fail(SAGNN_ERR_NULL, "edge drop: the sagnn_edge_drop is NULL");
  if (drop->keep_threshold == 0) return sagnn::fail(SAGNN_ERR_ARG, "edge drop: keep_threshold = 0 keeps no edge");
  if (!(drop->scale > 0.f) || !(drop->scale <= FLT_MAX))
    return sagnn::fail(SAGNN_ERR_ARG, "edge drop: scale = %g, need a finite value > 0", (double)drop->scale);
  if (n_layers > kDropMaxLayers)
    return sagnn::fail(SAGNN_ERR_ARG, "edge drop: n_layers = %d, the tag holds %d", n_layers, kDropMaxLayers);
  if (last_interval < 0 || last_interval >= kDropMaxIntervals)
    return sagnn::fail(SAGNN_ERR_ARG, "edge drop: interval %lld outside [0, 2^23)", (long long)last_interval);
  return SAGNN_OK;
}

RowDrop row_drop(const sagnn_edge_drop& e, uint32_t tag, bool rows_users) {
  return RowDrop{(uint32_t)e.seed, (uint32_t)(e.seed >> 32), e.step, e.keep_threshold, tag, rows_users ? 1 : 0, e.scale};
}
}

extern "C" int sagnn_spmm_drop_f32(const sagnn_spmm_plan* plan, const float* X, int64_t ldx, int d,
                                   const sagnn_spmm_epilogue* e, const sagnn_edge_drop* drop, uint32_t tag,
                                   int rows_are_users, void* workspace, size_t workspace_bytes, void* stream) {
  if (int rc = check_drop(drop, 0, 0)) return rc;
  if (!plan || !e) return sagnn::fail(SAGNN_ERR_NULL, "plan/epilogue is NULL");
  const RowDrop dr = row_drop(*drop, tag, rows_are_users != 0);
  return spmm_ex(plan, X, ldx, d, kernel_epilogue(*e, d), workspace, workspace_bytes, stream, &dr);
}

extern "C" int sagnn_spmm_f32(const sagnn_spmm_plan* plan, const float* X, int64_t ldx, int d,
                              const float* residual, int64_t ldr, float leaky, float* out,
                              int64_t ldo, const float* acc_in, int64_t ld_acc_in, float* acc_out,
                              int64_t ld_acc_out, void* workspace, size_t workspace_bytes,
                              void* stream) {
  sagnn_spmm_epilogue e{};
  e.leaky = leaky;
  e.residual = residual;
  e.ldr = ldr;
  e.out = out;
  e.ldo = ldo;
  e.acc_in = acc_in;
  e.ld_acc_in = ld_acc_in;
  e.acc_out = acc_out;
  e.ld_acc_out = ld_acc_out;
  return sagnn_spmm_ex_f32(plan, X, ldx, d, &e, workspace, workspace_bytes, stream);
}

extern "C" int sagnn_mask_scale_f32(const float* g, int64_t ldg, const uint8_t* mask, float slope, float* out, int64_t ldo,
                                    int64_t n_rows, int d, void* stream) {
  if (!g || !mask || !out) return sagnn::fail(SAGNN_ERR_NULL, "null pointer");
  if (int rc = check_d(d)) return rc;
  if (n_rows < 0) return sagnn::fail(SAGNN_ERR_ARG, "n_rows = %lld", (long long)n_rows);
  if (int rc = check_mat("g", g, ldg, d, true)) return rc;
  if (int rc = check_mat("out", out, ldo, d, true)) return rc;
  return launch_mask_scale(Slab{const_cast<float*>(g), ldg, 0}, mask, 0, slope, Slab{out, ldo, 0}, n_rows, d, 1,
                           static_cast<hipStream_t>(stream));
}

namespace {
int check_interval_plans(const sagnn_spmm_plan* pu, const sagnn_spmm_plan* pi) {
  if (!pu || !pi) return sagnn::fail(SAGNN_ERR_NULL, "plan is NULL");
  if (pu->info.n_src != pi->info.n_rows || pi->info.n_src != pu->info.n_rows)
    return sagnn::fail(SAGNN_ERR_ARG, "plans are not a transposed pair: user %lldx%lld, item %lldx%lld",
                       (long long)pu->info.n_rows, (long long)pu->info.n_src, (long long)pi->info.n_rows,
                       (long long)pi->info.n_src);
  return SAGNN_OK;
}
}

struct sagnn_spmm_batch {
  int T = 0;
  int64_t U = 0, I = 0;
  int64_t n_chunks = 0, n_long = 0, nnz = 0;
  SegMeta* d_meta = nullptr;
  const float** d_weights = nullptr;
  const uint16_t** d_buckets = nullptr;
  int32_t n_buckets = 0;
  int32_t* d_ints = nullptr;
  const int32_t *d_chunk_e0 = nullptr, *d_chunk_e1 = nullptr, *d_chunk_seg = nullptr, *d_long_row = nullptr,
                *d_long_seg = nullptr, *d_long_slot = nullptr, *d_chunk_row = nullptr;
};

namespace {
int batch_create(const sagnn_spmm_plan* const* plans_user, const sagnn_spmm_plan* const* plans_item, int n_intervals,
                 bool paired, sagnn_spmm_batch** batch_out) {
  if (!batch_out) return sagnn::fail(SAGNN_ERR_NULL, "batch_out is NULL");
  *batch_out = nullptr;
  if (!plans_user || !plans_item) return sagnn::fail(SAGNN_ERR_NULL, "plan table is NULL");
  if (n_intervals < 1 || n_intervals > 4096) return sagnn::fail(SAGNN_ERR_ARG, "n_intervals = %d", n_intervals);
  const int T = n_intervals;
  for (int k = 0; k < T; ++k) {
    if (paired) {
      if (int rc = check_interval_plans(plans_user[k], plans_item[k])) return rc;
    } else {
      if (!plans_user[k] || !plans_item[k]) return sagnn::fail(SAGNN_ERR_NULL, "plan is NULL");
      if (plans_user[k]->info.n_rows != plans_item[k]->info.n_rows || plans_user[k]->info.n_src != plans_user[0]->info.n_src ||
          plans_item[k]->info.n_src != plans_item[0]->info.n_src)
        return sagnn::fail(SAGNN_ERR_ARG, "interval %d: time-adjoint plans need one bucket count and one source row count per side", k);
    }
    if (!plans_user[k]->info.on_device || !plans_item[k]->info.on_device)
      return sagnn::fail(SAGNN_ERR_ARG, "interval %d: plan was built host-only", k);
    if (plans_user[k]->info.n_rows != plans_user[0]->info.n_rows || plans_item[k]->info.n_rows != plans_item[0]->info.n_rows)
      return sagnn::fail(SAGNN_ERR_ARG, "interval %d: every interval must have the same user / item counts", k);
  }
  const bool weighted = plans_user[0]->d_weights != nullptr;
  int32_t n_buckets = plans_user[0]->n_buckets;
  for (int k = 0; k < T; ++k)
    for (const sagnn_spmm_plan* p : {plans_user[k], plans_item[k]}) {
      if ((p->d_weights != nullptr) != weighted)
        return sagnn::fail(SAGNN_ERR_ARG, "interval %d: some plans of the batch carry edge weights and others do not "
                           "(sagnn_spmm_plan_set_weights): give all 2 T plans weights or none", k);
      if (p->n_buckets != n_buckets) n_buckets = 0;
    }
  sagnn_spmm_batch* b = new (std::nothrow) sagnn_spmm_batch();
  if (!b) return sagnn::fail(SAGNN_ERR_NOMEM, "out of host memory");
  b->T = T;
  b->U = plans_user[0]->info.n_rows;
  b->I = plans_item[0]->info.n_rows;
  std::vector<SegMeta> meta(2 * (size_t)T);
  std::vector<const float*> wtab(2 * (size_t)T);
  std::vector<const uint16_t*> btab(2 * (size_t)T);
  b->n_buckets = n_buckets;
  std::vector<int32_t> ce0, ce1, cseg, crow, lrow, lseg, lslot;
  try {
    for (int s = 0; s < 2 * T; ++s) {
      const sagnn_spmm_plan* p = s < T ? plans_user[s] : plans_item[s - T];
      meta[s] = SegMeta{p->d_rowptr, p->d_colidx, p->info.short_thresh, p->info.long_thresh};
      wtab[s] = p->d_weights;
      btab[s] = p->d_buckets;
      const int32_t coff = (int32_t)ce0.size();
      ce0.insert(ce0.end(), p->chunk_e0.begin(), p->chunk_e0.end());
      ce1.insert(ce1.end(), p->chunk_e1.begin(), p->chunk_e1.end());
      cseg.insert(cseg.end(), p->chunk_e0.size(), (int32_t)s);
      crow.insert(crow.end(), p->chunk_row.begin(), p->chunk_row.end());
      for (size_t j = 0; j < p->long_row.size(); ++j) {
        lrow.push_back(p->long_row[j]);
        lseg.push_back((int32_t)s);
        lslot.push_back(coff + p->long_slot[j]);
      }
      b->nnz += p->info.nnz;
    }
    lslot.push_back((int32_t)ce0.size());
  } catch (const std::bad_alloc&) {
    delete b;
    return sagnn::fail(SAGNN_ERR_NOMEM, "out of host memory building the batch tables");
  }
  if (ce0.size() > (size_t)INT32_MAX - 256) {
    delete b;
    return sagnn::fail(SAGNN_ERR_ARG, "too many long-row chunks for one batch");
  }
  b->n_chunks = (int64_t)ce0.size();
  b->n_long = (int64_t)lrow.size();
  hipError_t e = hipMalloc((void**)&b->d_meta, meta.size() * sizeof(SegMeta));
  if (e == hipSuccess) e = hipMemcpy(b->d_meta, meta.data(), meta.size() * sizeof(SegMeta), hipMemcpyHostToDevice);
  if (e == hipSuccess && weighted) {
    e = hipMalloc((void**)&b->d_weights, wtab.size() * sizeof(const float*));
    if (e == hipSuccess) e = hipMemcpy(b->d_weights, wtab.data(), wtab.size() * sizeof(const float*), hipMemcpyHostToDevice);
  }
  if (e == hipSuccess && n_buckets > 0) {
    e = hipMalloc((void**)&b->d_buckets, btab.size() * sizeof(const uint16_t*));
    if (e == hipSuccess) e = hipMemcpy(b->d_buckets, btab.data(), btab.size() * sizeof(const uint16_t*), hipMemcpyHostToDevice);
  }
  if (e == hipSuccess && b->n_chunks > 0) {
    const size_t nck = ce0.size(), nl = lrow.size();
    std::vector<int32_t> host;
    host.reserve(4 * nck + 3 * nl + 1);
    host.insert(host.end(), ce0.begin(), ce0.end());
    host.insert(host.end(), ce1.begin(), ce1.end());
    host.insert(host.end(), cseg.begin(), cseg.end());
    host.insert(host.end(), lrow.begin(), lrow.end());
    host.insert(host.end(), lseg.begin(), lseg.end());
    host.insert(host.end(), lslot.begin(), lslot.end());
    host.insert(host.end(), crow.begin(), crow.end());
    e = hipMalloc((void**)&b->d_ints, host.size() * sizeof(int32_t));
    if (e == hipSuccess) e = hipMemcpy(b->d_ints, host.data(), host.size() * sizeof(int32_t), hipMemcpyHostToDevice);
    b->d_chunk_e0 = b->d_ints;
    b->d_chunk_e1 = b->d_ints + nck;
    b->d_chunk_seg = b->d_ints + 2 * nck;
    b->d_long_row = b->d_ints + 3 * nck;
    b->d_long_seg = b->d_ints + 3 * nck + nl;
    b->d_long_slot = b->d_ints + 3 * nck + 2 * nl;
    b->d_chunk_row = b->d_ints + 3 * nck + 3 * nl + 1;
  }
  if (e != hipSuccess) {
    if (b->d_meta) (void)hipFree(b->d_meta);
    if (b->d_weights) (void)hipFree(b->d_weights);
    if (b->d_buckets) (void)hipFree(b->d_buckets);
    if (b->d_ints) (void)hipFree(b->d_ints);
    delete b;
    return sagnn::hip_fail(e, "batch tables (hipMalloc / hipMemcpy)");
  }
  *batch_out = b;
  return SAGNN_OK;
}
}

extern "C" int sagnn_spmm_batch_create(const sagnn_spmm_plan* const* plans_user, const sagnn_spmm_plan* const* plans_item,
                                       int n_intervals, sagnn_spmm_batch** batch_out) {
  return batch_create(plans_user, plans_item, n_intervals, true, batch_out);
}

extern "C" int sagnn_spmm_time_batch_create(const sagnn_spmm_plan* const* adj_user, const sagnn_spmm_plan* const* adj_item,
                                            int n_intervals, sagnn_spmm_batch** batch_out) {
  return batch_create(adj_user, adj_item, n_intervals, false, batch_out);
}

extern "C" int sagnn_spmm_batch_destroy(sagnn_spmm_batch* b) {
  if (!b) return SAGNN_OK;
  if (b->d_meta) (void)hipFree(b->d_meta);
  if (b->d_weights) (void)hipFree(b->d_weights);
  if (b->d_buckets) (void)hipFree(b->d_buckets);
  if (b->d_ints) (void)hipFree(b->d_ints);
  delete b;
  return SAGNN_OK;
}

extern "C" size_t sagnn_spmm_batch_workspace_bytes(const sagnn_spmm_batch* b, int d) {
  if (!b || d <= 0) return 0;
  return (size_t)b->n_chunks * (size_t)d * sizeof(float);
}

namespace {

template <int LPR>
int launch_batch(const sagnn_spmm_batch* b, int d, const DirArgs& au, const DirArgs& ai, float* partial, hipStream_t stream,
                 const BatchDrop* drop, const BatchTime* time) {
  constexpr int G = kWave / LPR;
  constexpr int RPW_SMALL = G > 4 ? G : 4;
  const bool small = (b->U > b->I ? b->U : b->I) < kSmallRows;
  const int64_t rpb = (int64_t)kWavesPerBlock * (small ? RPW_SMALL : kRowsPerWave);
  const int64_t chunk_blocks = (b->n_chunks + kWavesPerBlock - 1) / kWavesPerBlock;
  const int64_t bu = (b->U + rpb - 1) / rpb, bi = (b->I + rpb - 1) / rpb;
  const int64_t blocks = chunk_blocks + (int64_t)b->T * (bu + bi);
  if (blocks > INT32_MAX || b->U > INT32_MAX || b->I > INT32_MAX) return sagnn::fail(SAGNN_ERR_ARG, "grid too large");
  const BatchGeom g{b->T, (int32_t)chunk_blocks, (int32_t)bu, (int32_t)bi, (int32_t)b->U, (int32_t)b->I};
  if (blocks > 0) {
    sagnn::ProfileScope prof(sagnn::kProfSpmmRows, stream, b->nnz, (int64_t)b->T * (b->U + b->I));
    const auto rows = [&](auto kernel, auto... da) {
      hipLaunchKernelGGL(kernel, dim3((unsigned)blocks), dim3(kBlock), 0, stream, b->d_meta, g, b->d_chunk_e0, b->d_chunk_e1,
                         b->d_chunk_seg, b->n_chunks, partial, d, au, ai, da...);
    };
    const float* const* w = b->d_weights;
    if (time && w)
      rows(small ? spmm_rows_batch_kernel<LPR, RPW_SMALL, BatchTime, const float* const*>
                 : spmm_rows_batch_kernel<LPR, kRowsPerWave, BatchTime, const float* const*>, *time, w);
    else if (time)
      rows(small ? spmm_rows_batch_kernel<LPR, RPW_SMALL, BatchTime> : spmm_rows_batch_kernel<LPR, kRowsPerWave, BatchTime>, *time);
    else if (drop && w)
      rows(small ? spmm_rows_batch_kernel<LPR, RPW_SMALL, const int32_t*, BatchDrop, const float* const*>
                 : spmm_rows_batch_kernel<LPR, kRowsPerWave, const int32_t*, BatchDrop, const float* const*>,
           b->d_chunk_row, *drop, w);
    else if (drop)
      rows(small ? spmm_rows_batch_kernel<LPR, RPW_SMALL, const int32_t*, BatchDrop>
                 : spmm_rows_batch_kernel<LPR, kRowsPerWave, const int32_t*, BatchDrop>,
           b->d_chunk_row, *drop);
    else if (w)
      rows(small ? spmm_rows_batch_kernel<LPR, RPW_SMALL, const float* const*>
                 : spmm_rows_batch_kernel<LPR, kRowsPerWave, const float* const*>, w);
    else
      rows(small ? spmm_rows_batch_kernel<LPR, RPW_SMALL> : spmm_rows_batch_kernel<LPR, kRowsPerWave>);
    SAGNN_HIP_TRY(hipGetLastError());
  }
  if (b->n_long > 0) {
    sagnn::ProfileScope prof(sagnn::kProfSpmmFixup, stream, b->n_chunks, b->n_long);
    const int64_t fb = (b->n_long + kWavesPerBlock - 1) / kWavesPerBlock;
    const auto fixup = [&](auto kernel, auto... scale) {
      hipLaunchKernelGGL(kernel, dim3((unsigned)fb), dim3(kBlock), 0, stream,
                         b->d_long_row, b->d_long_slot, b->d_long_seg, b->n_long, partial, d, b->T, au, ai, scale...);
    };
    if (drop) fixup(spmm_fixup_batch_kernel<LPR, float>, drop->r.scale);
    else fixup(spmm_fixup_batch_kernel<LPR>);
    SAGNN_HIP_TRY(hipGetLastError());
  }
  return SAGNN_OK;
}

int launch_batch_d(const sagnn_spmm_batch* b, int d, const DirArgs& au, const DirArgs& ai, float* partial, hipStream_t s,
                   const BatchDrop* drop = nullptr, const BatchTime* time = nullptr) {
  switch (sagnn::lanes_per_row(d)) {
    case 8: return launch_batch<8>(b, d, au, ai, partial, s, drop, time);
    case 16: return launch_batch<16>(b, d, au, ai, partial, s, drop, time);
    case 32: return launch_batch<32>(b, d, au, ai, partial, s, drop, time);
    default: return launch_batch<64>(b, d, au, ai, partial, s, drop, time);
  }
}


int check_batch_ws(const sagnn_spmm_batch* b, int d, const void* workspace, size_t workspace_bytes) {
  const size_t need = sagnn_spmm_batch_workspace_bytes(b, d);
  if (need == 0) return SAGNN_OK;
  if (!workspace || workspace_bytes < need)
    return sagnn::fail(SAGNN_ERR_WORKSPACE, "workspace needs %zu bytes, got %zu", need, workspace ? workspace_bytes : (size_t)0);
  if (!sagnn::aligned16(workspace)) return sagnn::fail(SAGNN_ERR_ALIGN, "workspace not 16-byte aligned");
  return SAGNN_OK;
}

struct Side {
  Slab in, out;
  float* scratch;
  uint8_t* mask;
  int64_t rows;
};
struct Stack {
  Side u, i;
  int64_t T;
  int d, n_layers;
  float leaky;
};

Slab scratch_slot(const Stack& st, const Side& s, int slot) {
  return Slab{s.scratch + slot * st.T * s.rows * st.d, (int64_t)st.d, s.rows * st.d};
}

int check_stack(const Stack& st, bool scratch_used, const char* in_u, const char* in_i, const char* out_u, const char* out_i) {
  if (int rc = check_slab(in_u, st.u.in, st.d)) return rc;
  if (int rc = check_slab(in_i, st.i.in, st.d)) return rc;
  if (int rc = check_slab(out_u, st.u.out, st.d)) return rc;
  if (int rc = check_slab(out_i, st.i.out, st.d)) return rc;
  if (scratch_used && (!sagnn::aligned16(st.u.scratch) || !sagnn::aligned16(st.i.scratch)))
    return sagnn::fail(SAGNN_ERR_ALIGN, "scratch buffers must be 16-byte aligned");
  return SAGNN_OK;
}

DirArgs forward_layer(const Stack& st, const Side& self, const Side& other, int l) {
  const bool last = (l + 1 == st.n_layers);
  const int64_t mrow = st.d / 4;
  const Slab cur = l == 0 ? self.in : scratch_slot(st, self, (l - 1) & 1);
  const Slab x = l == 0 ? other.in : scratch_slot(st, other, (l - 1) & 1);
  DirArgs a{};
  a.ep.leaky = st.leaky;
  a.ep.mask_stride = (int)mrow;
  a.X = x.p, a.ldx = x.ld, a.s_X = x.slab;
  a.ep.residual = cur.p, a.ep.ldr = cur.ld, a.s_res = cur.slab;
  if (!last) {
    const Slab next = scratch_slot(st, self, l & 1);
    a.ep.out = next.p, a.ep.ldo = next.ld, a.s_out = next.slab;
  }
  if (last || l >= 1) {
    const Slab acc = l <= 1 ? cur : self.out;
    a.ep.acc_in = acc.p, a.ep.ld_acc_in = acc.ld, a.s_acc_in = acc.slab;
    a.ep.acc_out = self.out.p, a.ep.ld_acc_out = self.out.ld, a.s_acc_out = self.out.slab;
    if (last && l >= 1) a.ep.acc_in2 = self.in.p, a.ep.ld_acc_in2 = self.in.ld, a.s_acc_in2 = self.in.slab;
  }
  if (self.mask) {
    a.ep.mask_out = self.mask + (int64_t)l * self.rows * mrow;
    a.s_mask_out = (int64_t)st.n_layers * self.rows * mrow;
  }
  return a;
}

DirArgs backward_step(const Stack& st, const Side& self, const Side& other, int l) {
  const int L = st.n_layers;
  const int64_t mrow = st.d / 4;
  const int cur = (L - 1 - l) & 1;
  const Slab x = scratch_slot(st, other, 2 + cur);
  const Slab g_next = (l == L - 1) ? self.in : scratch_slot(st, self, (l + 1) & 1);
  const Slab g = (l == 0) ? self.out : scratch_slot(st, self, l & 1);
  DirArgs a{};
  a.ep.leaky = 1.f;
  a.ep.mask_stride = (int)mrow;
  a.X = x.p, a.ldx = x.ld, a.s_X = x.slab;
  a.ep.residual = g_next.p, a.ep.ldr = g_next.ld, a.s_res = g_next.slab;
  a.ep.acc_in = self.in.p, a.ep.ld_acc_in = self.in.ld, a.s_acc_in = self.in.slab;
  a.ep.acc_out = g.p, a.ep.ld_acc_out = g.ld, a.s_acc_out = g.slab;
  if (l > 0) {
    const Slab gm = scratch_slot(st, self, 2 + (cur ^ 1));
    a.ep.mask_in = self.mask + (int64_t)(l - 1) * self.rows * mrow;
    a.s_mask_in = (int64_t)L * self.rows * mrow;
    a.ep.out2 = gm.p, a.ep.ldo2 = gm.ld, a.s_out2 = gm.slab;
    a.ep.slope2 = st.leaky;
  }
  return a;
}

struct LayerTags {
  uint32_t tag_u, tag_i;
  int layer;
};

template <class Launch>
int run_forward(const Stack& st, Launch launch) {
  for (int l = 0; l < st.n_layers; ++l)
    if (int rc = launch(forward_layer(st, st.u, st.i, l), forward_layer(st, st.i, st.u, l),
                        LayerTags{(uint32_t)l << 1, (uint32_t)l << 1 | 1u, l}))
      return rc;
  return SAGNN_OK;
}

struct NoBeforeStep {
  int operator()(int, const Slab&, const Slab&) const { return SAGNN_OK; }
};
template <class Launch, class BeforeStep = NoBeforeStep>
int run_backward(const Stack& st, Launch launch, void* stream, BeforeStep before_step = BeforeStep{}) {
  for (const Side* s : {&st.u, &st.i}) {
    const int64_t mrow = st.d / 4;
    if (int rc = launch_mask_scale(s->in, s->mask + (int64_t)(st.n_layers - 1) * s->rows * mrow, st.n_layers * s->rows * mrow,
                                   st.leaky, scratch_slot(st, *s, 2), s->rows, st.d, st.T, static_cast<hipStream_t>(stream)))
      return rc;
  }
  for (int l = st.n_layers - 1; l >= 0; --l) {
    const int cur = (st.n_layers - 1 - l) & 1;
    if (int rc = before_step(l, scratch_slot(st, st.u, 2 + cur), scratch_slot(st, st.i, 2 + cur))) return rc;
    if (int rc = launch(backward_step(st, st.u, st.i, l), backward_step(st, st.i, st.u, l),
                        LayerTags{(uint32_t)l << 1 | 1u, (uint32_t)l << 1, l}))
      return rc;
  }
  return SAGNN_OK;
}

auto batched(const sagnn_spmm_batch* b, int d, void* workspace, void* stream) {
  return [=](const DirArgs& au, const DirArgs& ai, const LayerTags&) {
    return launch_batch_d(b, d, au, ai, static_cast<float*>(workspace), static_cast<hipStream_t>(stream));
  };
}

auto batched_drop(const sagnn_spmm_batch* b, int d, void* workspace, void* stream, const sagnn_edge_drop& drop) {
  return [=](const DirArgs& au, const DirArgs& ai, const LayerTags& t) {
    const BatchDrop bd{row_drop(drop, t.tag_u, true), t.tag_i};
    return launch_batch_d(b, d, au, ai, static_cast<float*>(workspace), static_cast<hipStream_t>(stream), &bd);
  };
}

auto per_plan(const sagnn_spmm_plan* plan_user, const sagnn_spmm_plan* plan_item, int d, void* workspace,
              size_t workspace_bytes, void* stream) {
  return [=](const DirArgs& au, const DirArgs& ai, const LayerTags&) {
    if (int rc = spmm_ex(plan_user, au.X, au.ldx, d, au.ep, workspace, workspace_bytes, stream)) return rc;
    return spmm_ex(plan_item, ai.X, ai.ldx, d, ai.ep, workspace, workspace_bytes, stream);
  };
}

auto per_plan_drop(const sagnn_spmm_plan* plan_user, const sagnn_spmm_plan* plan_item, int d, void* workspace,
                   size_t workspace_bytes, void* stream, const sagnn_edge_drop& drop, int interval) {
  return [=](const DirArgs& au, const DirArgs& ai, const LayerTags& t) {
    const uint32_t k = (uint32_t)interval << 8;
    const RowDrop du = row_drop(drop, t.tag_u | k, true), di = row_drop(drop, t.tag_i | k, false);
    if (int rc = spmm_ex(plan_user, au.X, au.ldx, d, au.ep, workspace, workspace_bytes, stream, &du)) return rc;
    return spmm_ex(plan_item, ai.X, ai.ldx, d, ai.ep, workspace, workspace_bytes, stream, &di);
  };
}

int check_time(const sagnn_edge_time* t, const sagnn_edge_drop* drop, int32_t n_buckets, int d) {
  if (drop) return sagnn::fail(SAGNN_ERR_ARG, "edge time: edge dropout and time do not combine (drop must be NULL)");
  if (!t || !t->te) return sagnn::fail(SAGNN_ERR_NULL, "edge time: the sagnn_edge_time or its te is NULL");
  if (n_buckets == 0) return sagnn::fail(SAGNN_ERR_ARG, "edge time: the plans carry no buckets (sagnn_spmm_plan_set_buckets)");
  if (t->n_buckets != n_buckets)
    return sagnn::fail(SAGNN_ERR_ARG, "edge time: n_buckets = %d but the plans were given %d", t->n_buckets, n_buckets);
  if (!sagnn::aligned16(t->te) || ((t->stride_interval | t->stride_layer | t->stride_dir) & 3) || (d & 3))
    return sagnn::fail(SAGNN_ERR_ALIGN, "edge time: te must be 16-byte aligned and its strides multiples of 4");
  return SAGNN_OK;
}

int check_time_bwd(const sagnn_edge_time* t, bool stack, int64_t U, int64_t I, int T) {
  if (!t->dte) return sagnn::fail(SAGNN_ERR_NULL, "edge time: dte is NULL");
  if (!sagnn::aligned16(t->dte)) return sagnn::fail(SAGNN_ERR_ALIGN, "edge time: dte must be 16-byte aligned");
  if (stack) {
    const sagnn_spmm_batch* b = t->adj_batch;
    if (!b) return sagnn::fail(SAGNN_ERR_NULL, "edge time: adj_batch is NULL");
    if (b->T != T || b->U != t->n_buckets || b->I != t->n_buckets)
      return sagnn::fail(SAGNN_ERR_ARG, "edge time: adj_batch is not the time batch of %d intervals and %d buckets", T, t->n_buckets);
    return SAGNN_OK;
  }
  if (!t->adj_user || !t->adj_item) return sagnn::fail(SAGNN_ERR_NULL, "edge time: adj_user / adj_item is NULL");
  if (t->adj_user->info.n_rows != t->n_buckets || t->adj_item->info.n_rows != t->n_buckets || t->adj_user->info.n_src != U ||
      t->adj_item->info.n_src != I)
    return sagnn::fail(SAGNN_ERR_ARG, "edge time: adj_user / adj_item are not %d x %lld and %d x %lld", t->n_buckets,
                       (long long)U, t->n_buckets, (long long)I);
  return SAGNN_OK;
}

auto per_plan_time(const sagnn_spmm_plan* plan_user, const sagnn_spmm_plan* plan_item, int d, void* workspace,
                   size_t workspace_bytes, void* stream, const sagnn_edge_time& tm, int interval) {
  return [=](const DirArgs& au, const DirArgs& ai, const LayerTags& t) {
    const float* te = tm.te + interval * tm.stride_interval + t.layer * tm.stride_layer;
    if (int rc = spmm_ex(plan_user, au.X, au.ldx, d, au.ep, workspace, workspace_bytes, stream, nullptr, te)) return rc;
    return spmm_ex(plan_item, ai.X, ai.ldx, d, ai.ep, workspace, workspace_bytes, stream, nullptr, te + tm.stride_dir);
  };
}

auto batched_time(const sagnn_spmm_batch* b, int d, void* workspace, void* stream, const sagnn_edge_time& tm) {
  return [=](const DirArgs& au, const DirArgs& ai, const LayerTags& t) {
    const BatchTime bt{b->d_buckets, tm.te + t.layer * tm.stride_layer, tm.stride_interval, tm.stride_dir};
    return launch_batch_d(b, d, au, ai, static_cast<float*>(workspace), static_cast<hipStream_t>(stream), nullptr, &bt);
  };
}

DirArgs dte_args(const Slab& gm, float* out, int d, int64_t s_out) {
  DirArgs a{};
  a.ep.leaky = 1.f;
  a.ep.mask_stride = d / 4;
  a.X = gm.p, a.ldx = gm.ld, a.s_X = gm.slab;
  a.ep.out = out, a.ep.ldo = d, a.s_out = s_out;
  return a;
}

auto dte_per_plan(const sagnn_edge_time& tm, int d, int interval, void* stream) {
  return [=](int l, const Slab& gm_u, const Slab& gm_i) {
    float* dte = tm.dte + interval * tm.stride_interval + l * tm.stride_layer;
    if (int rc = spmm_ex(tm.adj_user, gm_u.p, gm_u.ld, d, dte_args(gm_u, dte, d, 0).ep, tm.adj_workspace,
                         tm.adj_workspace_bytes, stream))
      return rc;
    return spmm_ex(tm.adj_item, gm_i.p, gm_i.ld, d, dte_args(gm_i, dte + tm.stride_dir, d, 0).ep, tm.adj_workspace,
                   tm.adj_workspace_bytes, stream);
  };
}

auto dte_batched(const sagnn_edge_time& tm, int d, void* stream) {
  return [=](int l, const Slab& gm_u, const Slab& gm_i) {
    float* dte = tm.dte + l * tm.stride_layer;
    return launch_batch_d(tm.adj_batch, d, dte_args(gm_u, dte, d, tm.stride_interval),
                          dte_args(gm_i, dte + tm.stride_dir, d, tm.stride_interval), static_cast<float*>(tm.adj_workspace),
                          static_cast<hipStream_t>(stream));
  };
}

Slab slab(const float* p, int64_t ld, int64_t stride) { return Slab{const_cast<float*>(p), ld, stride}; }

struct Graphs {
  const sagnn_spmm_plan *plan_user, *plan_item;
  const sagnn_spmm_batch* batch;
  bool stack;
  bool given() const { return stack ? batch != nullptr : plan_user && plan_item; }
  int64_t T() const { return stack ? batch->T : 1; }
  int64_t U() const { return stack ? batch->U : plan_user->info.n_rows; }
  int64_t I() const { return stack ? batch->I : plan_item->info.n_rows; }
};

int check_graphs(const Graphs& g) {
  if (g.stack) return g.batch ? SAGNN_OK : sagnn::fail(SAGNN_ERR_NULL, "batch is NULL");
  return check_interval_plans(g.plan_user, g.plan_item);
}

int check_form(const Graphs& g, const sagnn_gnn_args* a, bool backward) {
  if (!a) return sagnn::fail(SAGNN_ERR_NULL, "the sagnn_gnn_args is NULL");
  switch (a->edges) {
    case SAGNN_EDGES_PLAIN:
      if (a->drop || a->time) return sagnn::fail(SAGNN_ERR_ARG, "edges = SAGNN_EDGES_PLAIN with a drop or time struct");
      return SAGNN_OK;
    case SAGNN_EDGES_DROP:
      return check_drop(a->drop, a->n_layers, !g.stack ? a->interval : g.batch ? g.batch->T - 1 : 0);
    case SAGNN_EDGES_TIME: {
      if (!g.given()) return sagnn::fail(SAGNN_ERR_NULL, g.stack ? "batch is NULL" : "plan is NULL");
      int32_t n_buckets = a->time ? a->time->n_buckets : 0;
      if (!backward) {
        if (!g.stack && g.plan_user->n_buckets != g.plan_item->n_buckets)
          return sagnn::fail(SAGNN_ERR_ARG, "edge time: the two plans carry different bucket counts (or only one carries buckets)");
        n_buckets = g.stack ? g.batch->n_buckets : g.plan_user->n_buckets;
      }
      if (int rc = check_time(a->time, a->drop, n_buckets, a->d)) return rc;
      if (!g.stack && a->interval < 0) return sagnn::fail(SAGNN_ERR_ARG, "edge time: interval = %d", a->interval);
      return backward ? check_time_bwd(a->time, g.stack, g.U(), g.I(), (int)g.T()) : SAGNN_OK;
    }
  }
  return sagnn::fail(SAGNN_ERR_ARG, "edges = %d: not a SAGNN_EDGES_* value", a->edges);
}

Stack make_stack(const Graphs& g, const sagnn_gnn_args& a) {
  const auto side = [&](const sagnn_gnn_side& s, int64_t rows) {
    return Side{slab(s.in, s.ld_in, g.stack ? s.slab_in : 0), slab(s.out, s.ld_out, g.stack ? s.slab_out : 0), s.scratch,
                s.mask, rows};
  };
  return Stack{side(a.user, g.U()), side(a.item, g.I()), g.T(), a.d, a.n_layers, a.leaky};
}

// ... 87 lines not shown
```

### sa-gnn_amd/ops.py

```python
from __future__ import annotations

import ctypes
import math

import numpy as np
import torch

from . import _lib
from ._lib import PlanInfo, Tuning, check

SUPPORTED_D = tuple(range(4, 257, 4))

ENGINES = {"f16x2": 0, "f32": 1, "valu": 2}


def set_engine(name: str) -> None:
    check(_lib.load().sagnn_set_engine(ENGINES[name]))


def get_engine() -> str:
    code = _lib.load().sagnn_get_engine()
    return next(k for k, v in ENGINES.items() if v == code)


def range_redo_count(reset: bool = False) -> int:
    n = ctypes.c_int64(0)
    check(_lib.load().sagnn_range_redo_count(ctypes.byref(n), 1 if reset else 0))
    return int(n.value)


class engine:

    def __init__(self, name: str):
        self.name = name

    def __enter__(self):
        self.prev = get_engine()
        set_engine(self.name)
        return self

    def __exit__(self, *exc):
        set_engine(self.prev)
        return False


def _stream() -> int:
    return torch._C._cuda_getCurrentRawStream(torch.cuda.current_device())


def _ptr(t: torch.Tensor | None) -> int | None:
    return None if t is None else t.data_ptr()


def _f32_rows(name: str, t: torch.Tensor | None, d: int, rows: int | None = None):
    if t is None:
        return 0
    if t.dtype != torch.float32 or not t.is_cuda:
        raise TypeError(f"{name}: expected a float32 device tensor, got {t.dtype} on {t.device}")
    if t.dim() != 2 or t.shape[1] != d or t.stride(1) != 1:
        raise ValueError(f"{name}: expected shape [rows, {d}] with unit inner stride, got "
                         f"{tuple(t.shape)} strides {t.stride()}")
    if rows is not None and t.shape[0] != rows:
        raise ValueError(f"{name}: expected {rows} rows, got {t.shape[0]}")
    return t.stride(0) if t.shape[0] > 1 else max(t.stride(0), d)


def _f32_flat(name: str, t: torch.Tensor, numel: int) -> int:
    if not isinstance(t, torch.Tensor) or t.dtype != torch.float32 or not t.is_cuda:
        raise TypeError(f"{name}: expected a float32 device tensor")
    if not t.is_contiguous() or t.numel() != numel:
        raise ValueError(f"{name}: expected {numel} contiguous elements, got shape {tuple(t.shape)} strides {t.stride()}")
    return _ptr_or_empty(t)


def _ptr_or_empty(t: torch.Tensor) -> int:
    return t.data_ptr() or _empty_ptr(t.device)


def _one_device(ref: torch.Tensor, **others):
    for name, t in others.items():
        if t is not None and t.device != ref.device:
            raise ValueError(f"{name} on {t.device}, expected {ref.device}")


def _check_weights(weights, nnz: int) -> torch.Tensor:
    w = torch.as_tensor(weights)
    if w.dtype != torch.float32:
        raise TypeError(f"weights must be float32, got {w.dtype}")
    if w.dim() != 1 or w.numel() != nnz:
        raise ValueError(f"weights: expected {nnz} values (one per stored edge, in colidx order), got shape {tuple(w.shape)}")
    w = w.detach().cpu()
    if not bool(torch.isfinite(w).all()):
        raise ValueError("weights: NaN or Inf among the edge weights")
    return w


MAX_BUCKETS = 65535


def check_n_buckets(n_buckets: int) -> int:
    n_buckets = int(n_buckets)
    if not 1 <= n_buckets <= MAX_BUCKETS:
        raise ValueError(f"edge time: {n_buckets} time buckets, the bucket ids are uint16 and the table holds at most "
                         f"{MAX_BUCKETS} rows: choose a larger --slot (days per bucket)")
    return n_buckets


def _check_buckets(buckets, n_buckets: int, nnz: int) -> torch.Tensor:
    n_buckets = check_n_buckets(n_buckets)
    b = np.asarray(buckets.detach().cpu().numpy() if isinstance(buckets, torch.Tensor) else buckets)
    if b.dtype != np.uint16:
        raise TypeError(f"buckets must be uint16, got {b.dtype}")
    if b.ndim != 1 or b.size != nnz:
        raise ValueError(f"buckets: expected {nnz} values (one per stored edge, in colidx order), got shape {b.shape}")
    if b.size and int(b.max()) >= n_buckets:
        raise ValueError(f"buckets: id {int(b.max())} outside [0, {n_buckets})")
    return torch.from_numpy(np.ascontiguousarray(b))


def time_adjoint_arrays(rowptr, buckets, n_buckets: int, weights=None):
    rowptr = np.asarray(rowptr, dtype=np.int64)
    b = np.asarray(buckets, dtype=np.int64)
    rows = np.repeat(np.arange(rowptr.size - 1, dtype=np.int32), np.diff(rowptr))
    order = np.argsort(b, kind="stable")
    rp = np.zeros(int(n_buckets) + 1, dtype=np.int64)
    np.cumsum(np.bincount(b, minlength=int(n_buckets)), out=rp[1:])
    w = None if weights is None else np.ascontiguousarray(np.asarray(weights, dtype=np.float32)[order])
    return rp.astype(np.int32), np.ascontiguousarray(rows[order]), w


class SpmmPlan:

    def __init__(self, rowptr, colidx, n_rows: int, n_src: int, device=None,
                 tuning: tuple[int, int, int] | None = None, validate: bool = True, weights=None, buckets=None,
                 n_buckets: int | None = None):
        lib = _lib.load()
        self._lib = lib
        self._h = ctypes.c_void_p()
        self.n_rows, self.n_src = int(n_rows), int(n_src)
        rp_t = torch.as_tensor(rowptr)
        ci_t = torch.as_tensor(colidx)
        if rp_t.dtype != torch.int32 or ci_t.dtype != torch.int32:
            raise TypeError("rowptr/colidx must be int32")
        if rp_t.numel() != self.n_rows + 1:
            raise ValueError(f"rowptr has {rp_t.numel()} entries, expected n_rows+1 = {self.n_rows + 1}")
        self.nnz = int(ci_t.numel())
        w_t = None if weights is None else _check_weights(weights, self.nnz)
        if w_t is not None and device is None:
            raise ValueError("weights: a host-only plan (device=None) takes no weights")
        if (buckets is None) != (n_buckets is None):
            raise ValueError("buckets: give buckets and n_buckets together")
        b_t = None if buckets is None else _check_buckets(buckets, n_buckets, self.nnz)
        if b_t is not None and device is None:
            raise ValueError("buckets: a host-only plan (device=None) takes no buckets")
        rp_h = rp_t.cpu().contiguous()
        self._rowptr_host = rp_h.numpy()
        if validate:
            ci_h = ci_t.cpu().contiguous()
            check(lib.sagnn_csr_check_host(rp_h.data_ptr(), ci_h.data_ptr(), self.n_rows, self.n_src,
                                           self.nnz))
        tun = None
        if tuning is not None:
            tun = Tuning(int(tuning[0]), int(tuning[1]), int(tuning[2]), 0)
        if device is None:
            self.rowptr = self.colidx = None
            d_rp = d_ci = None
        else:
            self.rowptr = rp_t.to(device).contiguous()
            self.colidx = ci_t.to(device).contiguous()
            if self.colidx.numel() == 0:
                self.colidx = torch.zeros(1, dtype=torch.int32, device=device)
            d_rp, d_ci = self.rowptr.data_ptr(), self.colidx.data_ptr()
        check(lib.sagnn_spmm_plan_create(rp_h.data_ptr(), d_rp, d_ci, self.n_rows, self.n_src,
                                         self.nnz, ctypes.byref(tun) if tun else None,
                                         ctypes.byref(self._h)))
        info = PlanInfo()
        check(lib.sagnn_spmm_plan_get_info(self._h, ctypes.byref(info)))
        self.info = info
        self.device = device
        self._ws: dict[int, torch.Tensor] = {}
        self.partner_adjoint: SpmmPlan | None = None
        self.weights = None
        if w_t is not None:
            self.weights = w_t.to(device).contiguous()
            if self.weights.numel() == 0:
                self.weights = torch.zeros(1, dtype=torch.float32, device=device)
            check(lib.sagnn_spmm_plan_set_weights(self._h, self.weights.data_ptr()))
            check(lib.sagnn_spmm_plan_get_info(self._h, ctypes.byref(info)))
        self.buckets, self.n_buckets = None, 0
        self._tuning = tuning
        self._time_adjoint: SpmmPlan | None = None
        if b_t is not None:
            self._buckets_host = b_t.numpy()
            self._weights_host = None if w_t is None else w_t.numpy()
            self.n_buckets = int(n_buckets)
            self.buckets = b_t.to(device).contiguous()
            if self.buckets.numel() == 0:
                self.buckets = torch.zeros(1, dtype=torch.uint16, device=device)
            check(lib.sagnn_spmm_plan_set_buckets(self._h, self.buckets.data_ptr(), self.n_buckets))

    @property
    def time_adjoint(self) -> "SpmmPlan":
        if self.buckets is None:
            raise ValueError("time_adjoint: the plan has no buckets")
        if self._time_adjoint is None:
            rp, ci, w = time_adjoint_arrays(self._rowptr_host, self._buckets_host, self.n_buckets, self._weights_host)
            self._time_adjoint = SpmmPlan(rp, ci, self.n_buckets, self.n_rows, device=self.device, tuning=self._tuning,
                                          validate=False, weights=w)
        return self._time_adjoint

    @property
    def weighted(self) -> bool:
        return self.weights is not None

    def __del__(self):
        h = getattr(self, "_h", None)
        if h is not None and h.value:
            self._lib.sagnn_spmm_plan_destroy(h)
            self._h = None

    @property
    def handle(self):
        return self._h

    def chunks(self):
        n = int(self.info.n_chunks)
        rows = np.empty(n, np.int32)
        e0 = np.empty(n, np.int32)
        e1 = np.empty(n, np.int32)
        check(self._lib.sagnn_spmm_plan_copy_chunks(self._h, rows.ctypes.data, e0.ctypes.data,
                                                    e1.ctypes.data, n))
        return rows, e0, e1

    def workspace_bytes(self, d: int) -> int:
        return int(self._lib.sagnn_spmm_workspace_bytes(self._h, int(d)))

    def workspace(self, d: int) -> torch.Tensor | None:
        need = self.workspace_bytes(d)
        if need == 0:
            return None
        ws = self._ws.get(d)
        if ws is None:
            ws = torch.empty(need // 4, dtype=torch.float32, device=self.device)
            self._ws[d] = ws
        return ws


def spmm(plan: SpmmPlan, x: torch.Tensor, leaky: float, residual: torch.Tensor | None = None,
         out: torch.Tensor | None = None, acc_in: torch.Tensor | None = None,
         acc_out: torch.Tensor | None = None, want_out: bool = True) -> torch.Tensor | None:
    d = int(x.shape[1])
    ldx = _f32_rows("x", x, d, plan.n_src)
    if out is None and want_out:
        out = torch.empty((plan.n_rows, d), dtype=torch.float32, device=x.device)
    ldr = _f32_rows("residual", residual, d, plan.n_rows)
    ldo = _f32_rows("out", out, d, plan.n_rows)
    ldai = _f32_rows("acc_in", acc_in, d, plan.n_rows)
    ldao = _f32_rows("acc_out", acc_out, d, plan.n_rows)
    ws = plan.workspace(d)
    check(plan._lib.sagnn_spmm_f32(plan.handle, _ptr(x), ldx, d, _ptr(residual), ldr, float(leaky),
                                   _ptr(out), ldo, _ptr(acc_in), ldai, _ptr(acc_out), ldao,
                                   _ptr(ws), 0 if ws is None else ws.numel() * 4, _stream()))
    return out


def _call(entry, args: tuple, form_args: tuple, ws):
    check(entry(*args, *form_args, _ptr(ws), 0 if ws is None else ws.numel() * 4, _stream()))


def spmm_ex(plan: SpmmPlan, x: torch.Tensor | None, leaky: float, residual=None, out=None, acc_in=None, acc_out=None,
            acc_in2=None, mask_out=None, mask_in=None, out2=None, slope2: float = 1.0, want_out: bool = False,
            _drop=None, _time=None):
    ref = next(t_ for t_ in (x, residual, out, acc_out, out2) if t_ is not None)
    d = int(ref.shape[1])
    if out is None and want_out:
        out = torch.empty((plan.n_rows, d), dtype=torch.float32, device=ref.device)
    e = _lib.SpmmEpilogue()
    e.leaky, e.slope2 = float(leaky), float(slope2)
    e.residual, e.ldr = _ptr(residual), _f32_rows("residual", residual, d, plan.n_rows)
    e.out, e.ldo = _ptr(out), _f32_rows("out", out, d, plan.n_rows)
    e.acc_in, e.ld_acc_in = _ptr(acc_in), _f32_rows("acc_in", acc_in, d, plan.n_rows)
    e.acc_out, e.ld_acc_out = _ptr(acc_out), _f32_rows("acc_out", acc_out, d, plan.n_rows)
    e.acc_in2, e.ld_acc_in2 = _ptr(acc_in2), _f32_rows("acc_in2", acc_in2, d, plan.n_rows)
    e.out2, e.ldo2 = _ptr(out2), _f32_rows("out2", out2, d, plan.n_rows)
    for name, m in (("mask_out", mask_out), ("mask_in", mask_in)):
        if m is not None:
            _masks(name, m, (plan.n_rows, d // 4))
    e.mask_out, e.mask_in = _ptr(mask_out), _ptr(mask_in)
    ldx = _f32_rows("x", x, d, plan.n_src) if x is not None else d
    ws = plan.workspace(d)
    entry, form_args = plan._lib.sagnn_spmm_ex_f32, ()
    if _drop is not None:
        drop, tag, rows_are_users = _drop
        entry, form_args = plan._lib.sagnn_spmm_drop_f32, (ctypes.byref(drop.struct()), tag, int(rows_are_users))
    if _time is not None:
        et = _EdgeTime(_te_table("te", _time.view(1, 1, *_time.shape) if _time.dim() == 2 else _time, (1, 1),
                                 plan.n_buckets, d), plan.n_buckets, stack=False)
        entry, form_args = plan._lib.sagnn_spmm_time_f32, (None, ctypes.byref(et.args))
    _call(entry, (plan.handle, _ptr(x), ldx, d, ctypes.byref(e)), form_args, ws)
    return out


class EdgeDrop:

    def __init__(self, seed: int, step: int, keep: float):
        keep = float(keep)
        if not 0.0 < keep <= 1.0:
            raise ValueError(f"EdgeDrop: keep = {keep}, need 0 < keep <= 1")
        if not 0 <= int(seed) < 2 ** 64 or not 0 <= int(step) < 2 ** 32:
            raise ValueError(f"EdgeDrop: seed = {seed}, step = {step}: need 0 <= seed < 2^64, 0 <= step < 2^32")
        self.seed, self.step, self.keep = int(seed), int(step), keep
        self.threshold = min(int(math.floor(keep * 2.0 ** 32)), 2 ** 32 - 1)
        self.scale = float(np.float32(1.0) / np.float32(keep))
        if self.threshold == 0:
            raise ValueError(f"EdgeDrop: keep = {keep} is below 2^-32: no edge would be kept")

    @classmethod
    def raw(cls, seed: int, step: int, threshold: int, scale: float) -> "EdgeDrop":
        self = cls(seed, step, 1.0)
        self.threshold, self.scale, self.keep = int(threshold), float(scale), int(threshold) / 2.0 ** 32
        return self

    def struct(self) -> "_lib.EdgeDropArgs":
        return _lib.EdgeDropArgs(self.seed, self.step, self.threshold, self.scale)


def edge_tag(interval: int, layer: int, direction: int) -> int:
    return (int(interval) << 8) | (int(layer) << 1) | int(direction)


def spmm_drop(plan: SpmmPlan, x: torch.Tensor | None, leaky: float, drop: EdgeDrop, tag: int, rows_are_users: bool,
              residual=None, out=None, acc_in=None, acc_out=None, acc_in2=None, mask_out=None, mask_in=None, out2=None,
              slope2: float = 1.0, want_out: bool = False):
    return spmm_ex(plan, x, leaky, residual, out, acc_in, acc_out, acc_in2, mask_out, mask_in, out2, slope2, want_out,
                   _drop=(drop, int(tag), bool(rows_are_users)))


def _te_table(name: str, te: torch.Tensor, lead: tuple, n_buckets: int, d: int) -> torch.Tensor:
    if te.dtype != torch.float32 or not te.is_cuda or tuple(te.shape) != (*lead, n_buckets, d) or not te.is_contiguous():
        raise ValueError(f"{name}: expected a contiguous float32 device tensor {[*lead, n_buckets, d]}, got "
                         f"{tuple(te.shape)} {te.dtype} on {te.device}")
    return te


def _need_buckets(what: str, n_buckets: int) -> int:
    if not n_buckets:
        raise ValueError(f"{what}: a time table was given but the plans carry no buckets (SpmmPlan(..., buckets=, n_buckets=))")
    return n_buckets


class _EdgeTime:

    def __init__(self, te: torch.Tensor, n_buckets: int, stack: bool, dte: torch.Tensor | None = None, adj=None, d: int = 0):
        a = _lib.EdgeTimeArgs()
        a.te, a.n_buckets = te.data_ptr(), int(n_buckets)
        a.stride_dir = te.stride(-3)
        a.stride_layer = te.stride(-4)
        a.stride_interval = te.stride(0) if stack else 0
        self.keep = [te, dte, adj]
        if dte is not None:
            a.dte = dte.data_ptr()
            if stack:
                a.adj_batch = adj.handle
                ws = adj.workspace(d)
            else:
                a.adj_user, a.adj_item = adj[0].handle, adj[1].handle
                ws = _interval_ws(adj[0], adj[1], d)
            self.keep.append(ws)
            a.adj_workspace, a.adj_workspace_bytes = _ptr(ws), 0 if ws is None else ws.numel() * 4
        self.args = a


def spmm_time(plan: SpmmPlan, x: torch.Tensor | None, leaky: float, te: torch.Tensor, residual=None, out=None, acc_in=None,
              acc_out=None, acc_in2=None, mask_out=None, mask_in=None, out2=None, slope2: float = 1.0,
              want_out: bool = False):
    if plan.buckets is None:
        raise ValueError("spmm_time: the plan has no buckets (SpmmPlan(..., buckets=, n_buckets=))")
    return spmm_ex(plan, x, leaky, residual, out, acc_in, acc_out, acc_in2, mask_out, mask_in, out2, slope2, want_out,
                   _time=te)


def mask_scale(g: torch.Tensor, mask: torch.Tensor, slope: float, out: torch.Tensor):
    rows, d = int(g.shape[0]), int(g.shape[1])
    _masks("mask", mask, (rows, d // 4))
    check(_lib.load().sagnn_mask_scale_f32(_ptr(g), _f32_rows("g", g, d, rows), _ptr(mask), float(slope), _ptr(out),
                                           _f32_rows("out", out, d, rows), rows, d, _stream()))
    return out


def _interval_ws(plan_user: SpmmPlan, plan_item: SpmmPlan, d: int):
    wu, wi = plan_user.workspace(d), plan_item.workspace(d)
    return wu if (wi is None or (wu is not None and wu.numel() >= wi.numel())) else wi


def _scratch(name: str, s: torch.Tensor | None, k: int, rows: int, d: int, device):
    if s is None:
        return torch.empty(k * rows * d, dtype=torch.float32, device=device)
    if s.dtype != torch.float32 or not s.is_contiguous() or s.numel() < k * rows * d:
        raise ValueError(f"{name}: need a contiguous float32 buffer of {k}*{rows}*{d} elements")
    return s


def _masks(name: str, m: torch.Tensor, shape: tuple):
    if m.dtype != torch.uint8 or not m.is_contiguous() or m.numel() != int(np.prod(shape)):
        raise ValueError(f"{name}: need a contiguous uint8 tensor {list(shape)}")
    return m


def _adjoint_pair(plan_user: SpmmPlan, plan_item: SpmmPlan):
    adj_u, adj_i = plan_user.partner_adjoint, plan_item.partner_adjoint
    if (adj_u is None) != (adj_i is None):
        raise ValueError("give the exact adjoint of both plans or of neither")
    if adj_u is not None:
        return adj_u, adj_i
    if plan_user.nnz != plan_item.nnz:
        raise ValueError(f"plans are not a transposed pair (nnz {plan_user.nnz} vs {plan_item.nnz}: duplicated stored "
                         "entries?) — build them with graph.interval_pair, which adds the exact adjoints")
    return plan_user, plan_item


def _gnn_args(user: tuple, item: tuple, d: int, n_layers: int, leaky: float, drop, interval: int, et, ws):
    if et is not None and drop is not None:
        raise ValueError("edge dropout and time do not combine: give `drop` or `time`, not both")
    a = _lib.GnnArgs()
    for side, (x, ld_in, slab_in, out, ld_out, slab_out, scratch, mask) in ((a.user, user), (a.item, item)):
        side.in_, side.ld_in, side.slab_in = _ptr(x), ld_in, slab_in
        side.out, side.ld_out, side.slab_out = _ptr(out), ld_out, slab_out
        side.scratch, side.mask = _ptr(scratch), _ptr(mask)
    a.d, a.n_layers, a.leaky = d, int(n_layers), float(leaky)
    a.workspace, a.workspace_bytes = _ptr(ws), 0 if ws is None else ws.numel() * 4
    if et is not None:
        a.edges, a.time = _lib.EDGES_TIME, ctypes.pointer(et.args)
    elif drop is not None:
        a.edges, a.drop, a.interval = _lib.EDGES_DROP, ctypes.pointer(drop.struct()), int(interval)
    return a


def gnn_interval(plan_user: SpmmPlan, plan_item: SpmmPlan, u0: torch.Tensor, i0: torch.Tensor,
                 n_layers: int, leaky: float, user_out: torch.Tensor, item_out: torch.Tensor,
                 scratch_u: torch.Tensor | None = None, scratch_i: torch.Tensor | None = None,
                 mask_u: torch.Tensor | None = None, mask_i: torch.Tensor | None = None,
                 drop: EdgeDrop | None = None, interval: int = 0, time: torch.Tensor | None = None):
    d = int(u0.shape[1])
    U, I = plan_user.n_rows, plan_item.n_rows
    ld_u0 = _f32_rows("u0", u0, d, U)
    ld_i0 = _f32_rows("i0", i0, d, I)
    ld_uo = _f32_rows("user_out", user_out, d, U)
    ld_io = _f32_rows("item_out", item_out, d, I)
    if n_layers > 1:
        scratch_u = _scratch("scratch_u", scratch_u, 2, U, d, u0.device)
        scratch_i = _scratch("scratch_i", scratch_i, 2, I, d, u0.device)
    if mask_u is not None:
        _masks("mask_u", mask_u, (n_layers, U, d // 4))
    if mask_i is not None:
        _masks("mask_i", mask_i, (n_layers, I, d // 4))
    ws = _interval_ws(plan_user, plan_item, d)
    et = None if time is None else _EdgeTime(
        _te_table("time", time, (n_layers, 2), _need_buckets("gnn_interval", plan_user.n_buckets), d), plan_user.n_buckets,
        stack=False)
    args = _gnn_args((u0, ld_u0, 0, user_out, ld_uo, 0, scratch_u, mask_u),
                     (i0, ld_i0, 0, item_out, ld_io, 0, scratch_i, mask_i), d, n_layers, leaky, drop, interval, et, ws)
    check(plan_user._lib.sagnn_gnn_interval_f32(plan_user.handle, plan_item.handle, ctypes.byref(args), _stream()))
    return user_out, item_out


def gnn_interval_bwd(plan_user: SpmmPlan, plan_item: SpmmPlan, grad_user_out: torch.Tensor,
                     grad_item_out: torch.Tensor, n_layers: int, leaky: float, mask_u: torch.Tensor,
                     mask_i: torch.Tensor, grad_u0: torch.Tensor | None = None,
                     grad_i0: torch.Tensor | None = None, scratch_u: torch.Tensor | None = None,
                     scratch_i: torch.Tensor | None = None, drop: EdgeDrop | None = None, interval: int = 0,
                     time: torch.Tensor | None = None, grad_time: torch.Tensor | None = None):
    d = int(grad_user_out.shape[1])
    U, I = plan_user.n_rows, plan_item.n_rows
    et = None
    if time is not None:
        M = _need_buckets("gnn_interval_bwd", plan_user.n_buckets)
        et = _EdgeTime(_te_table("time", time, (n_layers, 2), M, d), M, stack=False,
                       dte=_te_table("grad_time", grad_time, (n_layers, 2), M, d),
                       adj=(plan_user.time_adjoint, plan_item.time_adjoint), d=d)
    plan_user, plan_item = _adjoint_pair(plan_user, plan_item)
    ld_gu = _f32_rows("grad_user_out", grad_user_out, d, U)
    ld_gi = _f32_rows("grad_item_out", grad_item_out, d, I)
    dev = grad_user_out.device
    if grad_u0 is None:
        grad_u0 = torch.empty((U, d), dtype=torch.float32, device=dev)
    if grad_i0 is None:
        grad_i0 = torch.empty((I, d), dtype=torch.float32, device=dev)
    ld_du = _f32_rows("grad_u0", grad_u0, d, U)
    ld_di = _f32_rows("grad_i0", grad_i0, d, I)
    scratch_u = _scratch("scratch_u", scratch_u, 4, U, d, dev)
    scratch_i = _scratch("scratch_i", scratch_i, 4, I, d, dev)
    _masks("mask_u", mask_u, (n_layers, U, d // 4))
    _masks("mask_i", mask_i, (n_layers, I, d // 4))
    ws = _interval_ws(plan_user, plan_item, d)
    args = _gnn_args((grad_user_out, ld_gu, 0, grad_u0, ld_du, 0, scratch_u, mask_u),
                     (grad_item_out, ld_gi, 0, grad_i0, ld_di, 0, scratch_i, mask_i), d, n_layers, leaky, drop, interval, et, ws)
    check(plan_user._lib.sagnn_gnn_interval_bwd_f32(plan_user.handle, plan_item.handle, ctypes.byref(args), _stream()))
    return grad_u0, grad_i0


class SpmmBatch:

    def __init__(self, plans_user, plans_item, _time_batch: bool = False):
        if len(plans_user) != len(plans_item) or not plans_user:
            raise ValueError("one user-side and one item-side plan per interval")
        self.plans_user, self.plans_item = list(plans_user), list(plans_item)
        self.weighted = self.plans_user[0].weighted
        if any(p.weighted != self.weighted for p in self.plans_user + self.plans_item):
            raise ValueError("SpmmBatch: some plans carry edge weights and others do not; give all 2 T plans weights or none")
        counts = {p.n_buckets for p in self.plans_user + self.plans_item}
        self.n_buckets = counts.pop() if len(counts) == 1 else 0
        self.T, self.U, self.I = len(plans_user), plans_user[0].n_rows, plans_item[0].n_rows
        self.device = plans_user[0].device
        self._lib = _lib.load()
        self._h = ctypes.c_void_p()
        PU = (ctypes.c_void_p * self.T)(*[p.handle for p in self.plans_user])
        PI = (ctypes.c_void_p * self.T)(*[p.handle for p in self.plans_item])
        create = self._lib.sagnn_spmm_time_batch_create if _time_batch else self._lib.sagnn_spmm_batch_create
        check(create(PU, PI, self.T, ctypes.byref(self._h)))
        self._time_adjoint: SpmmBatch | None = None
        self.nnz = sum(p.nnz for p in self.plans_user) + sum(p.nnz for p in self.plans_item)
        self._ws: dict[int, torch.Tensor] = {}
        self._adjoint: SpmmBatch | None = None

    def __del__(self):
        h = getattr(self, "_h", None)
        if h is not None and h.value:
            self._lib.sagnn_spmm_batch_destroy(h)
            self._h = None

    @property
    def handle(self):
        return self._h

    def workspace(self, d: int):
# ... 1045 lines not shown
```

Before: 18.20 billion.

## Split long-row chunks by source-column blocks and order chunks by block

```diff
diff --git a/include/sagnn.h b/include/sagnn.h
--- a/include/sagnn.h
+++ b/include/sagnn.h
@@ -43,7 +43,7 @@
   int32_t short_thresh;
   int32_t long_thresh;
   int32_t chunk_edges;
-  int32_t reserved;
+  int32_t src_block_rows;
 } sagnn_spmm_tuning;
 
 typedef struct sagnn_spmm_plan_info {
@@ -54,6 +54,10 @@
   int32_t max_degree;
   int32_t on_device;
   int32_t weighted;
+  int32_t n_src_blocks;
+  int32_t src_block_rows;
+  int32_t min_piece;
+  int32_t reserved;
 } sagnn_spmm_plan_info;
 
 int sagnn_spmm_plan_create(const int32_t* h_rowptr, const int32_t* d_rowptr,
@@ -64,6 +68,8 @@
 int sagnn_spmm_plan_get_info(const sagnn_spmm_plan* plan, sagnn_spmm_plan_info* info);
 int sagnn_spmm_plan_copy_chunks(const sagnn_spmm_plan* plan, int32_t* rows, int32_t* e_begin,
                                 int32_t* e_end, int64_t cap);
+int sagnn_spmm_plan_copy_slots(const sagnn_spmm_plan* plan, int32_t* slots, int64_t cap);
+int sagnn_spmm_plan_set_min_piece(sagnn_spmm_plan* plan, int32_t min_piece);
 int sagnn_spmm_plan_set_weights(sagnn_spmm_plan* plan, const float* d_weights);
 size_t sagnn_spmm_workspace_bytes(const sagnn_spmm_plan* plan, int d);
 
diff --git a/sa-gnn_amd/_lib.py b/sa-gnn_amd/_lib.py
--- a/sa-gnn_amd/_lib.py
+++ b/sa-gnn_amd/_lib.py
@@ -16,7 +16,7 @@
 
 class Tuning(ctypes.Structure):
     _fields_ = [("short_thresh", c_int32), ("long_thresh", c_int32), ("chunk_edges", c_int32),
-                ("reserved", c_int32)]
+                ("src_block_rows", c_int32)]
 
 
 class SpmmEpilogue(ctypes.Structure):
@@ -55,7 +55,8 @@
     _fields_ = [("n_rows", c_int64), ("n_src", c_int64), ("nnz", c_int64),
                 ("n_long_rows", c_int64), ("n_chunks", c_int64), ("short_thresh", c_int32),
                 ("long_thresh", c_int32), ("chunk_edges", c_int32), ("max_degree", c_int32),
-                ("on_device", c_int32), ("weighted", c_int32)]
+                ("on_device", c_int32), ("weighted", c_int32), ("n_src_blocks", c_int32),
+                ("src_block_rows", c_int32), ("min_piece", c_int32), ("reserved", c_int32)]
 
 
 SIGNATURES = {
@@ -73,6 +74,8 @@
     "sagnn_spmm_plan_get_info": (c_int, [c_void_p, POINTER(PlanInfo)]),
     "sagnn_spmm_plan_set_weights": (c_int, [c_void_p, c_void_p]),
     "sagnn_spmm_plan_copy_chunks": (c_int, [c_void_p, c_void_p, c_void_p, c_void_p, c_int64]),
+    "sagnn_spmm_plan_copy_slots": (c_int, [c_void_p, c_void_p, c_int64]),
+    "sagnn_spmm_plan_set_min_piece": (c_int, [c_void_p, c_int32]),
     "sagnn_spmm_workspace_bytes": (c_size_t, [c_void_p, c_int]),
     "sagnn_spmm_f32": (c_int, [c_void_p, c_void_p, c_int64, c_int, c_void_p, c_int64, c_float,
                                c_void_p, c_int64, c_void_p, c_int64, c_void_p, c_int64, c_void_p,
diff --git a/sa-gnn_amd/csrc/spmm.hip b/sa-gnn_amd/csrc/spmm.hip
--- a/sa-gnn_amd/csrc/spmm.hip
+++ b/sa-gnn_amd/csrc/spmm.hip
@@ -147,6 +147,9 @@
 }
 __device__ __forceinline__ RowTime seg_time(const RowTime& t, int, int, int) { return t; }
 
+struct ChunkSlot {
+  const int32_t* slot;
+};
 template <class T>
 struct KernelArg { using type = T; };
 template <class T>
@@ -160,7 +163,8 @@
   static constexpr bool TIME = kHas<RowTime, A...> || kHas<BatchTime, A...>;
   static_assert(DROP == kHas<const int32_t*, A...>, "a drop comes with the rows of the chunks");
   static_assert(!(DROP && TIME), "there are no drop + time kernels");
-  static_assert(sizeof...(A) == 2 * DROP + WEIGHTED + TIME, "trailing arguments: a drop, weights, a time term");
+  static constexpr bool SLOT = kHas<ChunkSlot, A...>;
+  static_assert(sizeof...(A) == 2 * DROP + WEIGHTED + TIME + SLOT, "trailing arguments: a drop, weights, a time term, the slots");
 };
 template <class Want>
 __device__ __forceinline__ Want arg_of() { return Want{}; }
@@ -173,6 +177,11 @@
 __device__ __forceinline__ int chunk_row_of(int64_t ci, A... da) {
   if constexpr (Pack<A...>::DROP) return arg_of<const int32_t*, A...>(da...)[ci];
   else return 0;
+}
+template <class... A>
+__device__ __forceinline__ int64_t chunk_slot_of(int64_t ci, A... da) {
+  if constexpr (Pack<A...>::SLOT) return arg_of<ChunkSlot, A...>(da...).slot[ci];
+  else return ci;
 }
 template <class... A>
 __device__ __forceinline__ const float* weights_of(int seg, A... da) {
@@ -437,7 +446,7 @@
     const float4 s = wave_row_sum<LPR, false, DROP, WEIGHTED, TIME>(
         colidx, chunk_e0[ci], chunk_e1[ci], X, ldx, lane, grp, col, lane_on, arg_of<RowDrop, DropArgs...>(da...),
         chunk_row_of<DropArgs...>(ci, da...), weights_of<DropArgs...>(0, da...), arg_of<RowTime, DropArgs...>(da...), d);
-    if (grp == 0 && lane_on) st4(partial + ci * (int64_t)d + col, s);
+    if (grp == 0 && lane_on) st4(partial + chunk_slot_of<DropArgs...>(ci, da...) * (int64_t)d + col, s);
     return;
   }
 
@@ -523,7 +532,7 @@
         meta[seg].colidx, chunk_e0[ci], chunk_e1[ci], a.X + (int64_t)k * a.s_X, a.ldx, lane, grp, col, lane_on,
         seg_drop(arg_of<BatchDrop, DropArgs...>(da...), dir, k), chunk_row_of<DropArgs...>(ci, da...),
         weights_of<DropArgs...>(seg, da...), tm, d);
-    if (grp == 0 && lane_on) st4(partial + ci * (int64_t)d + col, s);
+    if (grp == 0 && lane_on) st4(partial + chunk_slot_of<DropArgs...>(ci, da...) * (int64_t)d + col, s);
     return;
   }
   int rb = (int)blockIdx.x - g.chunk_blocks;
@@ -573,9 +582,12 @@
   const int32_t* d_colidx = nullptr;
   std::vector<int32_t> chunk_row, chunk_e0, chunk_e1;
   std::vector<int32_t> long_row, long_slot;
+  std::vector<int32_t> chunk_slot;
+  std::vector<int32_t> long_e0, long_e1;
   int32_t* d_meta = nullptr;
   const int32_t *d_chunk_e0 = nullptr, *d_chunk_e1 = nullptr, *d_long_row = nullptr,
-                *d_long_slot = nullptr, *d_chunk_row = nullptr;
+                *d_long_slot = nullptr, *d_chunk_row = nullptr,
+                *d_chunk_slot = nullptr;
   const float* d_weights = nullptr;
   const uint16_t* d_buckets = nullptr;
   int32_t n_buckets = 0;
@@ -594,6 +606,167 @@
   if (rp[n_rows] != nnz)
     return sagnn::fail(SAGNN_ERR_CSR, "rowptr[n_rows] = %d but nnz = %lld", rp[n_rows],
                        (long long)nnz);
+  return SAGNN_OK;
+}
+
+constexpr int kDefaultSrcBlock = 262144;
+constexpr int kDefaultMinPiece = 16;
+constexpr int64_t kMaxCutTable = (int64_t)1 << 27;
+
+__global__ __launch_bounds__(kBlock) void spmm_block_cuts_kernel(const int32_t* __restrict__ rowptr,
+                                                                const int32_t* __restrict__ colidx,
+                                                                const int32_t* __restrict__ long_row, int32_t B, int32_t nb,
+                                                                int32_t* __restrict__ cuts, int32_t* __restrict__ unsorted) {
+  const int64_t li = blockIdx.x;
+  const int r = long_row[li];
+  const int b = rowptr[r], e = rowptr[r + 1];
+  bool bad = false;
+  for (int i = b + (int)threadIdx.x; i + 1 < e; i += kBlock) bad |= colidx[i] > colidx[i + 1];
+  if (bad) *unsorted = 1;
+  for (int k = threadIdx.x; k <= nb; k += kBlock) {
+    const int64_t want = (int64_t)k * B;
+    int lo = b, hi = e;
+    while (lo < hi) {
+      const int mid = lo + (hi - lo) / 2;
+      if (colidx[mid] < want) lo = mid + 1;
+      else hi = mid;
+    }
+    cuts[li * ((int64_t)nb + 1) + k] = lo;
+  }
+}
+
+template <class Push>
+void cut_balanced(int32_t b, int32_t e, int32_t chunk, Push push) {
+  const int32_t n = e - b;
+  const int32_t nck = (n + chunk - 1) / chunk;
+  int32_t len = (n + nck - 1) / nck;
+  len = (len + kWave - 1) / kWave * kWave;
+  for (int32_t s = b; s < e; s += len) push(s, std::min(e, s + len));
+}
+
+int block_cuts(const sagnn_spmm_plan* p, int32_t B, int32_t nb, std::vector<int32_t>& cuts, bool* sorted) {
+  const size_t nl = p->long_row.size();
+  const size_t n_cuts = nl * ((size_t)nb + 1);
+  cuts.resize(1 + n_cuts);
+  int32_t* d = nullptr;
+  hipError_t e = hipMalloc((void**)&d, (nl + 1 + n_cuts) * sizeof(int32_t));
+  if (e != hipSuccess) return sagnn::hip_fail(e, "hipMalloc(source-block cut table)");
+  e = hipMemcpy(d, p->long_row.data(), nl * sizeof(int32_t), hipMemcpyHostToDevice);
+  if (e == hipSuccess) e = hipMemset(d + nl, 0, sizeof(int32_t));
+  if (e == hipSuccess) {
+    hipLaunchKernelGGL(spmm_block_cuts_kernel, dim3((unsigned)nl), dim3(kBlock), 0, nullptr, p->d_rowptr, p->d_colidx, d, B, nb,
+                       d + nl + 1, d + nl);
+    e = hipGetLastError();
+  }
+  if (e == hipSuccess) e = hipMemcpy(cuts.data(), d + nl, (1 + n_cuts) * sizeof(int32_t), hipMemcpyDeviceToHost);
+  (void)hipFree(d);
+  if (e != hipSuccess) return sagnn::hip_fail(e, "source-block cut table (launch / copy)");
+  *sorted = cuts[0] == 0;
+  cuts.erase(cuts.begin());
+  return SAGNN_OK;
+}
+
+int build_chunks(sagnn_spmm_plan* p, int32_t min_piece) {
+  const int32_t chunk = p->info.chunk_edges;
+  const size_t nl = p->long_row.size();
+  const int64_t B = p->info.src_block_rows;
+  const int64_t nb = B > 0 ? (p->info.n_src + B - 1) / B : 1;
+  bool blocks = p->d_rowptr && nl > 0 && nb > 1 && (int64_t)nl * (nb + 1) <= kMaxCutTable;
+  std::vector<int32_t> row, e0, e1, slot, lslot, host;
+  try {
+    std::vector<int32_t> cuts, blk;
+    if (blocks) {
+      if (int rc = block_cuts(p, (int32_t)B, (int32_t)nb, cuts, &blocks)) return rc;
+    }
+    lslot.push_back(0);
+    for (size_t li = 0; li < nl; ++li) {
+      const int32_t r = p->long_row[li], b = p->long_e0[li], e = p->long_e1[li];
+      const auto push = [&](int32_t s, int32_t t, int32_t k) {
+        row.push_back(r);
+        e0.push_back(s);
+        e1.push_back(t);
+        if (blocks) blk.push_back(k);
+      };
+      if (!blocks) {
+        cut_balanced(b, e, chunk, [&](int32_t s, int32_t t) { push(s, t, 0); });
+      } else {
+        int32_t* c = cuts.data() + li * (size_t)(nb + 1);
+        c[0] = b;
+        c[nb] = e;
+        for (int64_t k = 1; k < nb; ++k) c[k] = std::min(std::max(c[k], c[k - 1]), e);
+        for (int64_t k = 0; k < nb;) {
+          if (c[k + 1] == c[k]) {
+            ++k;
+            continue;
+          }
+          const int32_t s = c[k];
+          int64_t k1 = k + 1;
+          while (c[k1] - s < min_piece && k1 < nb) ++k1;
+          const int32_t t = c[k1];
+          if (t - s <= chunk) {
+            push(s, t, (int32_t)k);
+          } else {
+            int64_t kk = k;
+            cut_balanced(s, t, chunk, [&](int32_t q, int32_t q1) {
+              while (c[kk + 1] <= q) ++kk;
+              push(q, q1, (int32_t)kk);
+            });
+          }
+          k = k1;
+        }
+      }
+      lslot.push_back((int32_t)row.size());
+    }
+    const size_t nck = row.size();
+    if (blocks) {
+      slot.resize(nck);
+      for (size_t i = 0; i < nck; ++i) slot[i] = (int32_t)i;
+      std::stable_sort(slot.begin(), slot.end(), [&](int32_t a, int32_t z) { return blk[a] < blk[z]; });
+      std::vector<int32_t> tmp(nck);
+      for (auto* v : {&row, &e0, &e1}) {
+        for (size_t i = 0; i < nck; ++i) tmp[i] = (*v)[slot[i]];
+        v->swap(tmp);
+      }
+    }
+    if (p->d_rowptr && nck > 0) {
+      host.reserve(4 * nck + 2 * nl + 1);
+      host.insert(host.end(), e0.begin(), e0.end());
+      host.insert(host.end(), e1.begin(), e1.end());
+      host.insert(host.end(), p->long_row.begin(), p->long_row.end());
+      host.insert(host.end(), lslot.begin(), lslot.end());
+      host.insert(host.end(), row.begin(), row.end());
+      host.insert(host.end(), slot.begin(), slot.end());
+    }
+  } catch (const std::bad_alloc&) {
+    return sagnn::fail(SAGNN_ERR_NOMEM, "out of host memory building chunk list");
+  }
+  const size_t nck = row.size();
+  int32_t* d_meta = nullptr;
+  if (!host.empty()) {
+    hipError_t e = hipMalloc((void**)&d_meta, host.size() * sizeof(int32_t));
+    if (e != hipSuccess) return sagnn::hip_fail(e, "hipMalloc(plan metadata)");
+    e = hipMemcpy(d_meta, host.data(), host.size() * sizeof(int32_t), hipMemcpyHostToDevice);
+    if (e != hipSuccess) {
+      (void)hipFree(d_meta);
+      return sagnn::hip_fail(e, "hipMemcpy(plan metadata)");
+    }
+  }
+  if (p->d_meta) (void)hipFree(p->d_meta);
+  p->d_meta = d_meta;
+  p->d_chunk_e0 = d_meta;
+  p->d_chunk_e1 = d_meta ? d_meta + nck : nullptr;
+  p->d_long_row = d_meta ? d_meta + 2 * nck : nullptr;
+  p->d_long_slot = d_meta ? d_meta + 2 * nck + nl : nullptr;
+  p->d_chunk_row = d_meta ? d_meta + 2 * nck + 2 * nl + 1 : nullptr;
+  p->d_chunk_slot = d_meta && blocks ? d_meta + 3 * nck + 2 * nl + 1 : nullptr;
+  p->chunk_row.swap(row);
+  p->chunk_e0.swap(e0);
+  p->chunk_e1.swap(e1);
+  p->chunk_slot.swap(slot);
+  p->long_slot.swap(lslot);
+  p->info.n_chunks = (int64_t)nck;
+  p->info.n_src_blocks = blocks ? (int32_t)nb : 1;
+  p->info.min_piece = min_piece;
   return SAGNN_OK;
 }
 }
@@ -634,23 +807,18 @@
   chunk = (chunk + kWave - 1) / kWave * kWave;
   if (long_t < short_t) long_t = short_t;
 
+  int64_t src_block = tuning && tuning->src_block_rows != 0 ? tuning->src_block_rows : kDefaultSrcBlock;
+  if (src_block < 0 || src_block >= n_src) src_block = 0;
+
   int32_t max_deg = 0;
   try {
-    p->long_slot.push_back(0);
     for (int64_t r = 0; r < n_rows; ++r) {
       const int32_t b = h_rowptr[r], e = h_rowptr[r + 1], deg = e - b;
       max_deg = std::max(max_deg, deg);
       if (deg <= long_t) continue;
-      const int32_t nck = (deg + chunk - 1) / chunk;
-      int32_t len = (deg + nck - 1) / nck;
-      len = (len + kWave - 1) / kWave * kWave;
-      for (int32_t s = b; s < e; s += len) {
-        p->chunk_row.push_back((int32_t)r);
-        p->chunk_e0.push_back(s);
-        p->chunk_e1.push_back(std::min(e, s + len));
-      }
       p->long_row.push_back((int32_t)r);
-      p->long_slot.push_back((int32_t)p->chunk_row.size());
+      p->long_e0.push_back(b);
+      p->long_e1.push_back(e);
     }
   } catch (const std::bad_alloc&) {
     delete p;
@@ -661,45 +829,39 @@
   p->info.n_src = n_src;
   p->info.nnz = nnz;
   p->info.n_long_rows = (int64_t)p->long_row.size();
-  p->info.n_chunks = (int64_t)p->chunk_row.size();
   p->info.short_thresh = short_t;
   p->info.long_thresh = long_t;
   p->info.chunk_edges = chunk;
   p->info.max_degree = max_deg;
-  p->info.on_device = 0;
+  p->info.on_device = d_rowptr ? 1 : 0;
+  p->info.src_block_rows = (int32_t)src_block;
   p->d_rowptr = d_rowptr;
   p->d_colidx = d_colidx;
-
-  if (d_rowptr) {
-    const size_t nck = p->chunk_row.size(), nl = p->long_row.size();
-    if (nck > 0) {
-      const size_t words = 3 * nck + nl + (nl + 1);
-      hipError_t e = hipMalloc((void**)&p->d_meta, words * sizeof(int32_t));
-      if (e != hipSuccess) {
-        delete p;
-        return sagnn::hip_fail(e, "hipMalloc(plan metadata)");
-      }
-      std::vector<int32_t> host(words);
-      std::copy(p->chunk_e0.begin(), p->chunk_e0.end(), host.begin());
-      std::copy(p->chunk_e1.begin(), p->chunk_e1.end(), host.begin() + nck);
-      std::copy(p->long_row.begin(), p->long_row.end(), host.begin() + 2 * nck);
-      std::copy(p->long_slot.begin(), p->long_slot.end(), host.begin() + 2 * nck + nl);
-      std::copy(p->chunk_row.begin(), p->chunk_row.end(), host.begin() + 2 * nck + 2 * nl + 1);
-      e = hipMemcpy(p->d_meta, host.data(), words * sizeof(int32_t), hipMemcpyHostToDevice);
-      if (e != hipSuccess) {
-        (void)hipFree(p->d_meta);
-        delete p;
-        return sagnn::hip_fail(e, "hipMemcpy(plan metadata)");
-      }
-      p->d_chunk_e0 = p->d_meta;
-      p->d_chunk_e1 = p->d_meta + nck;
-      p->d_long_row = p->d_meta + 2 * nck;
-      p->d_long_slot = p->d_meta + 2 * nck + nl;
-      p->d_chunk_row = p->d_meta + 2 * nck + 2 * nl + 1;
-    }
-    p->info.on_device = 1;
+  if (int rc = build_chunks(p, kDefaultMinPiece)) {
+    delete p;
+    return rc;
   }
   *plan_out = p;
+  return SAGNN_OK;
+}
+
+extern "C" int sagnn_spmm_plan_set_min_piece(sagnn_spmm_plan* plan, int32_t min_piece) {
+  if (!plan) return sagnn::fail(SAGNN_ERR_NULL, "plan is NULL");
+  if (min_piece < 0) return sagnn::fail(SAGNN_ERR_ARG, "min_piece = %d: need >= 0 (0 = default)", min_piece);
+  if (min_piece == 0) min_piece = kDefaultMinPiece;
+  if (min_piece == plan->info.min_piece) return SAGNN_OK;
+  return build_chunks(plan, min_piece);
+}
+
+extern "C" int sagnn_spmm_plan_copy_slots(const sagnn_spmm_plan* plan, int32_t* slots, int64_t cap) {
+  if (!plan) return sagnn::fail(SAGNN_ERR_NULL, "plan is NULL");
+  const int64_t n = plan->info.n_chunks;
+  if (cap < n) return sagnn::fail(SAGNN_ERR_ARG, "cap %lld < n_chunks %lld", (long long)cap, (long long)n);
+  if (n > 0 && !slots) return sagnn::fail(SAGNN_ERR_NULL, "null output array");
+  if (plan->chunk_slot.empty())
+    for (int64_t i = 0; i < n; ++i) slots[i] = (int32_t)i;
+  else
+    std::copy(plan->chunk_slot.begin(), plan->chunk_slot.end(), slots);
   return SAGNN_OK;
 }
 
@@ -772,29 +934,24 @@
   if (blocks > INT32_MAX) return sagnn::fail(SAGNN_ERR_ARG, "grid too large");
   if (blocks > 0) {
     sagnn::ProfileScope prof(sagnn::kProfSpmmRows, stream, p->info.nnz, n_rows);
-    const auto rows = [&](auto kernel, auto... da) {
+    const auto rows = [&](auto... da) {
+      const auto kernel = small ? spmm_rows_kernel<LPR, RPW_SMALL, decltype(da)...> : spmm_rows_kernel<LPR, kRowsPerWave, decltype(da)...>;
       hipLaunchKernelGGL(kernel, dim3((unsigned)blocks), dim3(kBlock), 0, stream, p->d_rowptr, p->d_colidx, X, ldx, d, n_rows,
                          p->info.short_thresh, p->info.long_thresh, p->d_chunk_e0, p->d_chunk_e1, n_chunks,
                          (int)chunk_blocks, partial, ep, da...);
     };
+    const auto form = [&](auto... da) {
+      if (p->d_chunk_slot) rows(da..., ChunkSlot{p->d_chunk_slot});
+      else rows(da...);
+    };
     const float* w = p->d_weights;
     const RowTime tm{p->d_buckets, te};
-    if (te && w)
-      rows(small ? spmm_rows_kernel<LPR, RPW_SMALL, RowTime, const float*> : spmm_rows_kernel<LPR, kRowsPerWave, RowTime, const float*>,
-           tm, w);
-    else if (te)
-      rows(small ? spmm_rows_kernel<LPR, RPW_SMALL, RowTime> : spmm_rows_kernel<LPR, kRowsPerWave, RowTime>, tm);
-    else if (drop && w)
-      rows(small ? spmm_rows_kernel<LPR, RPW_SMALL, const int32_t*, RowDrop, const float*>
-                 : spmm_rows_kernel<LPR, kRowsPerWave, const int32_t*, RowDrop, const float*>,
-           p->d_chunk_row, *drop, w);
-    else if (drop)
-      rows(small ? spmm_rows_kernel<LPR, RPW_SMALL, const int32_t*, RowDrop> : spmm_rows_kernel<LPR, kRowsPerWave, const int32_t*, RowDrop>,
-           p->d_chunk_row, *drop);
-    else if (w)
-      rows(small ? spmm_rows_kernel<LPR, RPW_SMALL, const float*> : spmm_rows_kernel<LPR, kRowsPerWave, const float*>, w);
-    else
-      rows(small ? spmm_rows_kernel<LPR, RPW_SMALL> : spmm_rows_kernel<LPR, kRowsPerWave>);
+    if (te && w) form(tm, w);
+    else if (te) form(tm);
+    else if (drop && w) form(p->d_chunk_row, *drop, w);
+    else if (drop) form(p->d_chunk_row, *drop);
+    else if (w) form(w);
+    else form();
     SAGNN_HIP_TRY(hipGetLastError());
   }
   const int64_t n_long = p->info.n_long_rows;
@@ -981,7 +1138,8 @@
   int32_t n_buckets = 0;
   int32_t* d_ints = nullptr;
   const int32_t *d_chunk_e0 = nullptr, *d_chunk_e1 = nullptr, *d_chunk_seg = nullptr, *d_long_row = nullptr,
-                *d_long_seg = nullptr, *d_long_slot = nullptr, *d_chunk_row = nullptr;
+                *d_long_seg = nullptr, *d_long_slot = nullptr, *d_chunk_row = nullptr,
+                *d_chunk_slot = nullptr;
 };
 
 namespace {
@@ -1024,7 +1182,9 @@
   std::vector<const float*> wtab(2 * (size_t)T);
   std::vector<const uint16_t*> btab(2 * (size_t)T);
   b->n_buckets = n_buckets;
-  std::vector<int32_t> ce0, ce1, cseg, crow, lrow, lseg, lslot;
+  std::vector<int32_t> ce0, ce1, cseg, crow, cslot, lrow, lseg, lslot;
+  bool slots = false;
+  for (int k = 0; k < T; ++k) slots = slots || !plans_user[k]->chunk_slot.empty() || !plans_item[k]->chunk_slot.empty();
   try {
     for (int s = 0; s < 2 * T; ++s) {
       const sagnn_spmm_plan* p = s < T ? plans_user[s] : plans_item[s - T];
@@ -1036,6 +1196,8 @@
       ce1.insert(ce1.end(), p->chunk_e1.begin(), p->chunk_e1.end());
       cseg.insert(cseg.end(), p->chunk_e0.size(), (int32_t)s);
       crow.insert(crow.end(), p->chunk_row.begin(), p->chunk_row.end());
+      if (slots)
+        for (size_t j = 0; j < p->chunk_e0.size(); ++j) cslot.push_back(coff + (p->chunk_slot.empty() ? (int32_t)j : p->chunk_slot[j]));
       for (size_t j = 0; j < p->long_row.size(); ++j) {
         lrow.push_back(p->long_row[j]);
         lseg.push_back((int32_t)s);
@@ -1067,7 +1229,7 @@
   if (e == hipSuccess && b->n_chunks > 0) {
     const size_t nck = ce0.size(), nl = lrow.size();
     std::vector<int32_t> host;
-    host.reserve(4 * nck + 3 * nl + 1);
+    host.reserve(5 * nck + 3 * nl + 1);
     host.insert(host.end(), ce0.begin(), ce0.end());
     host.insert(host.end(), ce1.begin(), ce1.end());
     host.insert(host.end(), cseg.begin(), cseg.end());
@@ -1075,6 +1237,7 @@
     host.insert(host.end(), lseg.begin(), lseg.end());
     host.insert(host.end(), lslot.begin(), lslot.end());
     host.insert(host.end(), crow.begin(), crow.end());
+    host.insert(host.end(), cslot.begin(), cslot.end());
     e = hipMalloc((void**)&b->d_ints, host.size() * sizeof(int32_t));
     if (e == hipSuccess) e = hipMemcpy(b->d_ints, host.data(), host.size() * sizeof(int32_t), hipMemcpyHostToDevice);
     b->d_chunk_e0 = b->d_ints;
@@ -1084,6 +1247,7 @@
     b->d_long_seg = b->d_ints + 3 * nck + nl;
     b->d_long_slot = b->d_ints + 3 * nck + 2 * nl;
     b->d_chunk_row = b->d_ints + 3 * nck + 3 * nl + 1;
+    if (slots) b->d_chunk_slot = b->d_ints + 4 * nck + 3 * nl + 1;
   }
   if (e != hipSuccess) {
     if (b->d_meta) (void)hipFree(b->d_meta);
@@ -1139,29 +1303,22 @@
   const BatchGeom g{b->T, (int32_t)chunk_blocks, (int32_t)bu, (int32_t)bi, (int32_t)b->U, (int32_t)b->I};
   if (blocks > 0) {
     sagnn::ProfileScope prof(sagnn::kProfSpmmRows, stream, b->nnz, (int64_t)b->T * (b->U + b->I));
-    const auto rows = [&](auto kernel, auto... da) {
+    const auto rows = [&](auto... da) {
+      const auto kernel = small ? spmm_rows_batch_kernel<LPR, RPW_SMALL, decltype(da)...> : spmm_rows_batch_kernel<LPR, kRowsPerWave, decltype(da)...>;
       hipLaunchKernelGGL(kernel, dim3((unsigned)blocks), dim3(kBlock), 0, stream, b->d_meta, g, b->d_chunk_e0, b->d_chunk_e1,
                          b->d_chunk_seg, b->n_chunks, partial, d, au, ai, da...);
     };
+    const auto form = [&](auto... da) {
+      if (b->d_chunk_slot) rows(da..., ChunkSlot{b->d_chunk_slot});
+      else rows(da...);
+    };
     const float* const* w = b->d_weights;
-    if (time && w)
-      rows(small ? spmm_rows_batch_kernel<LPR, RPW_SMALL, BatchTime, const float* const*>
-                 : spmm_rows_batch_kernel<LPR, kRowsPerWave, BatchTime, const float* const*>, *time, w);
-    else if (time)
-      rows(small ? spmm_rows_batch_kernel<LPR, RPW_SMALL, BatchTime> : spmm_rows_batch_kernel<LPR, kRowsPerWave, BatchTime>, *time);
-    else if (drop && w)
-      rows(small ? spmm_rows_batch_kernel<LPR, RPW_SMALL, const int32_t*, BatchDrop, const float* const*>
-                 : spmm_rows_batch_kernel<LPR, kRowsPerWave, const int32_t*, BatchDrop, const float* const*>,
-           b->d_chunk_row, *drop, w);
-    else if (drop)
-      rows(small ? spmm_rows_batch_kernel<LPR, RPW_SMALL, const int32_t*, BatchDrop>
-                 : spmm_rows_batch_kernel<LPR, kRowsPerWave, const int32_t*, BatchDrop>,
-           b->d_chunk_row, *drop);
-    else if (w)
-      rows(small ? spmm_rows_batch_kernel<LPR, RPW_SMALL, const float* const*>
-                 : spmm_rows_batch_kernel<LPR, kRowsPerWave, const float* const*>, w);
-    else
-      rows(small ? spmm_rows_batch_kernel<LPR, RPW_SMALL> : spmm_rows_batch_kernel<LPR, kRowsPerWave>);
+    if (time && w) form(*time, w);
+    else if (time) form(*time);
+    else if (drop && w) form(b->d_chunk_row, *drop, w);
+    else if (drop) form(b->d_chunk_row, *drop);
+    else if (w) form(w);
+    else form();
     SAGNN_HIP_TRY(hipGetLastError());
   }
   if (b->n_long > 0) {
diff --git a/sa-gnn_amd/ops.py b/sa-gnn_amd/ops.py
--- a/sa-gnn_amd/ops.py
+++ b/sa-gnn_amd/ops.py
@@ -132,7 +132,7 @@
 class SpmmPlan:
 
     def __init__(self, rowptr, colidx, n_rows: int, n_src: int, device=None,
-                 tuning: tuple[int, int, int] | None = None, validate: bool = True, weights=None, buckets=None,
+                 tuning: tuple[int, ...] | None = None, validate: bool = True, weights=None, buckets=None,
                  n_buckets: int | None = None):
         lib = _lib.load()
         self._lib = lib
@@ -160,8 +160,12 @@
             check(lib.sagnn_csr_check_host(rp_h.data_ptr(), ci_h.data_ptr(), self.n_rows, self.n_src,
                                            self.nnz))
         tun = None
+        min_piece = 0
         if tuning is not None:
-            tun = Tuning(int(tuning[0]), int(tuning[1]), int(tuning[2]), 0)
+            if not 3 <= len(tuning) <= 5:
+                raise ValueError("tuning: (short_thresh, long_thresh, chunk_edges[, src_block_rows[, min_piece]])")
+            tun = Tuning(int(tuning[0]), int(tuning[1]), int(tuning[2]), int(tuning[3]) if len(tuning) > 3 else 0)
+            min_piece = int(tuning[4]) if len(tuning) > 4 else 0
         if device is None:
             self.rowptr = self.colidx = None
             d_rp = d_ci = None
@@ -174,6 +178,8 @@
         check(lib.sagnn_spmm_plan_create(rp_h.data_ptr(), d_rp, d_ci, self.n_rows, self.n_src,
                                          self.nnz, ctypes.byref(tun) if tun else None,
                                          ctypes.byref(self._h)))
+        if min_piece:
+            check(lib.sagnn_spmm_plan_set_min_piece(self._h, min_piece))
         info = PlanInfo()
         check(lib.sagnn_spmm_plan_get_info(self._h, ctypes.byref(info)))
         self.info = info
@@ -231,6 +237,12 @@
         check(self._lib.sagnn_spmm_plan_copy_chunks(self._h, rows.ctypes.data, e0.ctypes.data,
                                                     e1.ctypes.data, n))
         return rows, e0, e1
+
+    def slots(self):
+        n = int(self.info.n_chunks)
+        slots = np.empty(n, np.int32)
+        check(self._lib.sagnn_spmm_plan_copy_slots(self._h, slots.ctypes.data, n))
+        return slots
 
     def workspace_bytes(self, d: int) -> int:
         return int(self._lib.sagnn_spmm_workspace_bytes(self._h, int(d)))
```

Result: no change. 18.30 billion (median of 5 runs) (+0.6%).
